# nyu-systems/Grendel-GS

Hardware: AMD Instinct MI355X
Metric: training iters/sec (fwd+bwd) (higher is better)
Workload: dtype f32

## Files before the change

### grendel-gs_amd/csrc/api.hip

```cpp
#include "common.h"

extern "C" {

const char *gsr_error_string(int code) {
    if (code == 0) return "success";
    if (code == GSR_EINVAL) return "gsraster: invalid argument";
    if (code == GSR_ENOSPACE) return "gsraster: workspace too small";
    if (code == GSR_ERETRY) return "gsraster: pair count valid, bounded sort must be repeated";
    if (code == GSR_EFAULT)
        return "gsraster: a persistent binning kernel of an earlier call timed out at a grid barrier (hung or preempted "
               "device); that view's lists are incomplete; the look-back pipeline is used from now on";
    if (code > 0) return hipGetErrorString((hipError_t)code);
    return "gsraster: unknown error";
}

int gsr_abi_version(void) { return 15; }

int gsr_get_block_xy(int *block_x, int *block_y, int *one_dim_block) {
    if (!block_x || !block_y || !one_dim_block) return GSR_EINVAL;
    *block_x = GSR_BLOCK_X;
    *block_y = GSR_BLOCK_Y;
    *one_dim_block = GSR_ONE_DIM_BLOCK;
    return 0;
}
// ... 98 lines not shown
    if (!xyz || !scaling || !rotation || !features_dc || !features_rest || !opacity || !viewmatrix || !projmatrix ||
        !campos || !radii || !cov3D || !clamped || !dL_dmeans2D || !dL_dconic_opacity || !dL_drgb || !dL_dxyz ||
        !dL_dscaling || !dL_drotation || !dL_dfeatures_dc || !dL_dfeatures_rest || !dL_dopacity)
        return GSR_EINVAL;
    return gsr_launch_preprocess_backward(P, sh_degree, sh_coeffs, xyz, scaling, scale_modifier, rotation, features_dc,
                                          features_rest, opacity, viewmatrix, projmatrix, campos, width, height,
                                          tanfovx, tanfovy, radii, cov3D, clamped, dL_dmeans2D, dL_dconic_opacity,
                                          dL_drgb, grad_row_stride, dL_dxyz, dL_dscaling, dL_drotation, dL_dfeatures_dc,
                                          dL_dfeatures_rest, dL_dopacity, gsr_antialiasing_mode(),
                                          reinterpret_cast<hipStream_t>(stream));
}

int gsr_get_local2j_ids_bool(int P, int width, int height, int world_size, const float *means2D,
                             const int32_t *radii, const int32_t *dist_global_strategy, uint8_t *out,
                             gsr_stream_t stream) {
    if (P < 0 || width <= 0 || height <= 0 || world_size <= 0) return GSR_EINVAL;
    if (P == 0) return 0;
    if (!means2D || !radii || !dist_global_strategy || !out) return GSR_EINVAL;
    return gsr_launch_local2j(P, width, height, world_size, means2D, radii, dist_global_strategy, out,
                              reinterpret_cast<hipStream_t>(stream));
}

size_t gsr_render_seg_bytes(int width, int height) {
    if (width <= 0 || height <= 0) return 0;
    return gsr_composite_seg_bytes(width, height);
}

int gsr_render_forward(int P, int width, int height, const int32_t *ranges, const uint32_t *point_list,
                       const float *means2D, const float *conic_opacity, const float *rgb,
                       const uint8_t *compute_locally, const float *bg, float *out_color, float *final_T,
                       int32_t *n_contrib, void *seg_ws, size_t seg_bytes, int row_lo, int row_hi, void *zero_ptr,
                       size_t zero_bytes, gsr_stream_t stream) {
    if (P < 0 || width <= 0 || height <= 0) return GSR_EINVAL;
    if (!ranges || !compute_locally || !bg || !out_color || !final_T || !n_contrib) return GSR_EINVAL;
    if (P > 0 && (!means2D || !conic_opacity || !rgb)) return GSR_EINVAL;
    return gsr_launch_composite_forward(P, width, height, ranges, point_list, means2D, conic_opacity, rgb,
                                        compute_locally, bg, out_color, final_T, n_contrib, seg_ws, seg_bytes, row_lo,
                                        row_hi, zero_ptr, zero_bytes, reinterpret_cast<hipStream_t>(stream));
}

int gsr_render_backward(int P, int width, int height, const int32_t *ranges, const uint32_t *point_list,
                        const float *means2D, const float *conic_opacity, const float *rgb,
                        const uint8_t *compute_locally, const float *bg, const float *final_T,
                        const int32_t *n_contrib, const float *dL_dpixels, float *dL_record, const float *out_color,
                        void *seg_ws, size_t seg_bytes, int row_lo, int row_hi, int record_is_zero, double *acc64,
                        uint8_t *touched, gsr_stream_t stream) {
    if (P < 0 || width <= 0 || height <= 0) return GSR_EINVAL;
    if (P == 0) return 0;
    if (!ranges || !compute_locally || !bg || !final_T || !n_contrib || !dL_dpixels || !means2D || !conic_opacity ||
        !rgb || !dL_record || !acc64)
        return GSR_EINVAL;
    return gsr_launch_composite_backward(P, width, height, ranges, point_list, means2D, conic_opacity, rgb,
                                         compute_locally, bg, final_T, n_contrib, dL_dpixels, dL_record, out_color,
                                         seg_ws, seg_bytes, row_lo, row_hi, record_is_zero ? 1 : 0, acc64, touched,
                                         reinterpret_cast<hipStream_t>(stream));
}

int gsr_render_contrib(int P, int width, int height, const int32_t *ranges, const uint32_t *point_list,
                       const float *means2D, const float *conic_opacity, const uint8_t *compute_locally,
                       const int32_t *n_contrib, int row_lo, int row_hi, int64_t *hits, float *wmax, double *wsum,
                       gsr_stream_t stream) {
    if (P < 0 || width <= 0 || height <= 0) return GSR_EINVAL;
    if (P == 0) return 0;
    if (!ranges || !means2D || !conic_opacity || !compute_locally || !n_contrib || !hits || !wmax || !wsum)
        return GSR_EINVAL;
    return gsr_launch_composite_contrib(P, width, height, ranges, point_list, means2D, conic_opacity, compute_locally,
                                        n_contrib, row_lo, row_hi, hits, wmax, wsum,
                                        reinterpret_cast<hipStream_t>(stream));
}

int gsr_contrib_merge_rows(int64_t n, const int32_t *idx, const int64_t *src_hits, const float *src_wmax,
                           const double *src_wsum, int64_t *dst_hits, float *dst_wmax, double *dst_wsum,
                           gsr_stream_t stream) {
    if (n < 0) return GSR_EINVAL;
    if (n == 0) return 0;
    if (!idx || !src_hits || !src_wmax || !src_wsum || !dst_hits || !dst_wmax || !dst_wsum) return GSR_EINVAL;
    return gsr_launch_contrib_merge_rows(n, idx, src_hits, src_wmax, src_wsum, dst_hits, dst_wmax, dst_wsum,
                                         reinterpret_cast<hipStream_t>(stream));
}

int gsr_render_invdepth(int P, int width, int height, const int32_t *ranges, const uint32_t *point_list,
                        const float *means2D, const float *conic_opacity, const float *depths,
                        const uint8_t *compute_locally, const int32_t *n_contrib, int row_lo, int row_hi,
                        float *invdepth, gsr_stream_t stream) {
    if (P < 0 || width <= 0 || height <= 0 || !invdepth) return GSR_EINVAL;
    if (P > 0 && (!ranges || !means2D || !conic_opacity || !depths || !compute_locally || !n_contrib)) return GSR_EINVAL;
    return gsr_launch_composite_invdepth(P, width, height, ranges, point_list, means2D, conic_opacity, depths,
                                         compute_locally, n_contrib, row_lo, row_hi, invdepth,
                                         reinterpret_cast<hipStream_t>(stream));
}

int gsr_render_invdepth_backward(int P, int width, int height, const int32_t *ranges, const uint32_t *point_list,
                                 const float *means2D, const float *conic_opacity, const float *depths,
                                 const uint8_t *compute_locally, const int32_t *n_contrib, const float *final_T,
                                 const float *invdepth, const float *dL_dinvdepth, int row_lo, int row_hi,
                                 float *dL_record, double *acc64, gsr_stream_t stream) {
    if (P < 0 || width <= 0 || height <= 0) return GSR_EINVAL;
    if (P == 0) return 0;
    if (!ranges || !means2D || !conic_opacity || !depths || !compute_locally || !n_contrib || !final_T || !invdepth ||
        !dL_dinvdepth || !dL_record || !acc64)
        return GSR_EINVAL;
    return gsr_launch_composite_invdepth_backward(P, width, height, ranges, point_list, means2D, conic_opacity, depths,
                                                  compute_locally, n_contrib, final_T, dL_dinvdepth, row_lo, row_hi,
                                                  dL_record, acc64, reinterpret_cast<hipStream_t>(stream));
}

int gsr_depth_backward_means3d(int P, const int32_t *radii, const float *viewmatrix, const float *dL_ddepth,
// ... 10 lines not shown
```

### grendel-gs_amd/csrc/common.h

```cpp
#pragma once
#include <hip/hip_runtime.h>
#include <stdint.h>

#include "../../include/gsraster.h"

#define GSR_WAVE 64

#define GSR_LAUNCH_CHECK()                         \
    do {                                           \
        hipError_t e__ = hipGetLastError();        \
        if (e__ != hipSuccess) return (int)e__;    \
    } while (0)

#define GSR_HIP(expr)                              \
    do {                                           \
        hipError_t e__ = (expr);                   \
        if (e__ != hipSuccess) return (int)e__;    \
    } while (0)

static inline int gsr_div_up(long long a, long long b) { return (int)((a + b - 1) / b); }

__device__ __forceinline__ int gsr_xcd_span_of_block(int b, int nwg) {
#ifdef GSR_NO_XCD_MAP
    return b;
// ... 59 lines not shown
__device__ __forceinline__ bool gsr_can_touch_box(const float2 xy, const float4 co, float x0, float y0, float x1,
                                                  float y1) {
    if (!(co.w >= 1.0f / 255.0f)) return false;
    const float lim = (2.0f * 0.6931471805599453f) * __builtin_amdgcn_logf(255.0f * co.w) * 1.002f + 0.01f;
    const float l = x0 - xy.x, r = x1 - xy.x, t = y0 - xy.y, bt = y1 - xy.y;
    if (l <= 0.f && r >= 0.f && t <= 0.f && bt >= 0.f) return true;
    if (!(co.x > 0.f && co.z > 0.f)) return true;
    const float rcz = __builtin_amdgcn_rcpf(co.z), rcx = __builtin_amdgcn_rcpf(co.x);
    float q = gsr_edge_min_q(co.x, co.y, co.z, rcz, l, t, bt);
    q = fminf(q, gsr_edge_min_q(co.x, co.y, co.z, rcz, r, t, bt));
    q = fminf(q, gsr_edge_min_q(co.z, co.y, co.x, rcx, t, l, r));
    q = fminf(q, gsr_edge_min_q(co.z, co.y, co.x, rcx, bt, l, r));
    return !(q > lim);
}

__device__ __forceinline__ void gsr_adam1(float &p, float g, float &m, float &v, float lr_c, float b1, float b2,
                                          float omb1, float omb2, float inv_sqrt_bc2, float eps) {
    m = __builtin_fmaf(b1, m, __fmul_rn(omb1, g));
    v = __builtin_fmaf(b2, v, __fmul_rn(__fmul_rn(omb2, g), g));
    const float denom = __builtin_fmaf(__fsqrt_rn(v), inv_sqrt_bc2, eps);
    p = __builtin_fmaf(-lr_c, __fdiv_rn(m, denom), p);
}

int gsr_launch_preprocess_forward(int P, int D, int M, const float *means3D, const float *scales, float scale_modifier,
                                  const float *rotations, const float *shs, const float *shs_rest,
                                  const float *opacities,
                                  const float *viewmatrix, const float *projmatrix, const float *campos, int W, int H,
                                  float tanfovx, float tanfovy, float *means2D, float *depths, int32_t *radii,
                                  float *cov3D, float *conic_opacity, float *rgb, uint8_t *clamped, int aa,
                                  hipStream_t stream);
int gsr_launch_preprocess_backward(int P, int D, int M, const float *means3D, const float *scales,
                                   float scale_modifier, const float *rotations, const float *shs,
                                   const float *shs_rest, const float *opacities_raw, const float *viewmatrix, const float *projmatrix, const float *campos, int W,
                                   int H, float tanfovx, float tanfovy, const int32_t *radii, const float *cov3D,
                                   const uint8_t *clamped, const float *dL_dmeans2D, const float *dL_dconic_opacity,
                                   const float *dL_drgb, int grad_row_stride, float *dL_dmeans3D, float *dL_dscales, float *dL_drotations,
                                   float *dL_dshs, float *dL_dshs_rest, float *dL_dopacities, int aa,
                                   hipStream_t stream);
int gsr_antialiasing_mode();
int gsr_launch_local2j(int P, int W, int H, int ws, const float *means2D, const int32_t *radii, const int32_t *div,
                       uint8_t *out, hipStream_t stream);

int gsr_launch_composite_forward(int P, int W, int H, const int32_t *ranges, const uint32_t *point_list,
                                 const float *means2D, const float *conic_opacity, const float *rgb,
                                 const uint8_t *compute_locally, const float *bg, float *out_color, float *final_T,
                                 int32_t *n_contrib, void *seg_ws, size_t seg_bytes, int row_lo, int row_hi,
                                 void *zero_ptr, size_t zero_bytes, hipStream_t stream);
size_t gsr_composite_seg_bytes(int W, int H);
int gsr_launch_composite_backward(int P, int W, int H, const int32_t *ranges, const uint32_t *point_list,
                                  const float *means2D, const float *conic_opacity, const float *rgb,
                                  const uint8_t *compute_locally, const float *bg, const float *final_T,
                                  const int32_t *n_contrib, const float *dL_dpixels, float *dL_record,
                                  const float *out_color, void *seg_ws, size_t seg_bytes, int row_lo, int row_hi,
                                  int record_is_zero, double *acc64, uint8_t *touched, hipStream_t stream);
int gsr_launch_composite_contrib(int P, int W, int H, const int32_t *ranges, const uint32_t *point_list,
                                 const float *means2D, const float *conic_opacity, const uint8_t *compute_locally,
                                 const int32_t *n_contrib, int row_lo, int row_hi, int64_t *hits, float *wmax,
                                 double *wsum, hipStream_t stream);
int gsr_launch_contrib_merge_rows(int64_t n, const int32_t *idx, const int64_t *src_hits, const float *src_wmax,
                                  const double *src_wsum, int64_t *dst_hits, float *dst_wmax, double *dst_wsum,
                                  hipStream_t stream);
int gsr_launch_composite_invdepth(int P, int W, int H, const int32_t *ranges, const uint32_t *point_list,
                                  const float *means2D, const float *conic_opacity, const float *depths,
                                  const uint8_t *compute_locally, const int32_t *n_contrib, int row_lo, int row_hi,
                                  float *invdepth, hipStream_t stream);
int gsr_launch_composite_invdepth_backward(int P, int W, int H, const int32_t *ranges, const uint32_t *point_list,
                                           const float *means2D, const float *conic_opacity, const float *depths,
                                           const uint8_t *compute_locally, const int32_t *n_contrib,
                                           const float *final_T, const float *dL_dinvdepth, int row_lo, int row_hi,
                                           float *dL_record, double *acc64, hipStream_t stream);
int gsr_launch_depth_to_means3D(int P, const int32_t *radii, const float *viewmatrix, const float *dL_ddepth,
                                int row_stride, float *dL_dmeans3D, int overwrite, hipStream_t stream);
```

### grendel-gs_amd/csrc/composite.hip

```cpp
#include "common.h"
#include "composite_math.h"

namespace {

__device__ unsigned long long g_walked[2];

#ifdef GSR_STATS
__device__ unsigned long long g_stats[8];
#define GSR_STAT(i, v) do { const unsigned long long sv__ = (unsigned long long)(v); if (lane == 0) atomicAdd(&g_stats[i], sv__); } while (0)
#else
#define GSR_STAT(i, v) do { } while (0)
#endif

typedef float v2f __attribute__((ext_vector_type(2)));
constexpr int PREC = 20;
struct PairRec {
    v2f x, y, a2, b2, c2, o, r, g, b;
};
__device__ __forceinline__ void pair_store(float *__restrict__ slab, int pos, const Entry &e, float r, float g, float b) {
    float *rec = slab + (pos >> 1) * PREC + (pos & 1);
    rec[0] = e.x;  rec[2] = e.y;  rec[4] = e.a2;  rec[6] = e.b2;  rec[8] = e.c2;
    rec[10] = e.o; rec[12] = r;   rec[14] = g;    rec[16] = b;
}
__device__ __forceinline__ void pair_store_last(float *__restrict__ slab, int pos, int last) {
    slab[(pos >> 1) * PREC + 18 + (pos & 1)] = __int_as_float(last);
}
__device__ __forceinline__ PairRec pair_load_last(const float *__restrict__ slab, int pair, int &la, int &lb) {
    const float4 *q = reinterpret_cast<const float4 *>(slab + pair * PREC);
    const float4 q0 = q[0], q1 = q[1], q2 = q[2], q3 = q[3], q4 = q[4];
    PairRec p;
    p.x = v2f{q0.x, q0.y};  p.y = v2f{q0.z, q0.w};  p.a2 = v2f{q1.x, q1.y};  p.b2 = v2f{q1.z, q1.w};
    p.c2 = v2f{q2.x, q2.y}; p.o = v2f{q2.z, q2.w};  p.r = v2f{q3.x, q3.y};   p.g = v2f{q3.z, q3.w};
    p.b = v2f{q4.x, q4.y};
    la = __float_as_int(q4.z);
    lb = __float_as_int(q4.w);
    asm("" : "+v"(la), "+v"(lb));
    return p;
}
#ifdef GSR_LOG2O
#define GSR_PAD_O (-__builtin_inff())
#else
#define GSR_PAD_O 0.f
#endif
__device__ __forceinline__ PairRec pair_load(const float *__restrict__ slab, int pair) {
    const float4 *q = reinterpret_cast<const float4 *>(slab + pair * PREC);
    const float4 q0 = q[0], q1 = q[1], q2 = q[2], q3 = q[3];
    const float2 q4 = *reinterpret_cast<const float2 *>(q + 4);
    PairRec p;
    p.x = v2f{q0.x, q0.y};  p.y = v2f{q0.z, q0.w};  p.a2 = v2f{q1.x, q1.y};  p.b2 = v2f{q1.z, q1.w};
    p.c2 = v2f{q2.x, q2.y}; p.o = v2f{q2.z, q2.w};  p.r = v2f{q3.x, q3.y};   p.g = v2f{q3.z, q3.w};
    p.b = v2f{q4.x, q4.y};
    return p;
// ... 727 lines not shown

int gsr_launch_composite_forward(int P, int W, int H, const int32_t *ranges, const uint32_t *point_list,
                                 const float *means2D, const float *conic_opacity, const float *rgb,
                                 const uint8_t *compute_locally, const float *bg, float *out_color, float *final_T,
                                 int32_t *n_contrib, void *seg_ws, size_t seg_bytes, int row_lo, int row_hi,
                                 void *zero_ptr, size_t zero_bytes, hipStream_t stream) {
    (void)P;
    if (zero_bytes && (!zero_ptr || ((uintptr_t)zero_ptr & 15) || (zero_bytes & 3))) return GSR_EINVAL;
    const size_t zero16_n = zero_bytes / 16;
    if (zero_bytes & 15)
        GSR_HIP(hipMemsetAsync(reinterpret_cast<char *>(zero_ptr) + zero16_n * 16, 0, zero_bytes & 15, stream));
    const int gx = (W + GSR_BLOCK_X - 1) / GSR_BLOCK_X, gy = (H + GSR_BLOCK_Y - 1) / GSR_BLOCK_Y;
    const BandGrid b = band_grid_of(row_lo, row_hi, gx, gy);
    if (seg_ws && seg_bytes < seg_ws_bytes(gx * gy, SEG_CAP)) return GSR_ENOSPACE;
    const SegWs seg = seg_ws_of(seg_ws, gx * gy, SEG_CAP);
    if (seg_ws) GSR_HIP(hipMemsetAsync(seg_ws, 0, 64, stream));
    auto launch = [&](auto kern) {
        hipLaunchKernelGGL(kern, dim3(b.band ? b.band_tiles : gx * gy), dim3(256), 0, stream, W, H, gx,
                           reinterpret_cast<const int2 *>(ranges), point_list, reinterpret_cast<const float2 *>(means2D),
                           reinterpret_cast<const float4 *>(conic_opacity), rgb, compute_locally, bg, out_color, final_T,
                           n_contrib, seg, b.band_first, b.band_tiles, reinterpret_cast<uint4 *>(zero_ptr), zero16_n);
    };
    if (seg_ws && b.band) launch(composite_forward_kernel<true, true>);
    else if (seg_ws) launch(composite_forward_kernel<true, false>);
    else if (b.band) launch(composite_forward_kernel<false, true>);
    else launch(composite_forward_kernel<false, false>);
    GSR_LAUNCH_CHECK();
    return 0;
}

__global__ void record_from_f64_kernel(const double *__restrict__ acc, float *__restrict__ rec, size_t n) {
    const size_t i = (size_t)blockIdx.x * blockDim.x + threadIdx.x;
    if (i < n) rec[i] = (float)acc[i];
}

__global__ void record_from_f64_touched_kernel(const double *__restrict__ acc, float *__restrict__ rec,
                                               const uint8_t *__restrict__ touched, int P) {
    const int i = (int)(blockIdx.x * blockDim.x + threadIdx.x);
    if (i >= P || !touched[i]) return;
    const double *a = acc + 9 * (size_t)i;
    float *r = rec + 9 * (size_t)i;
    double v[9];
#pragma unroll
    for (int k = 0; k < 9; k++) v[k] = a[k];
#pragma unroll
    for (int k = 0; k < 9; k++) r[k] = (float)v[k];
}

int gsr_launch_composite_backward(int P, int W, int H, const int32_t *ranges, const uint32_t *point_list,
                                  const float *means2D, const float *conic_opacity, const float *rgb,
                                  const uint8_t *compute_locally, const float *bg, const float *final_T,
                                  const int32_t *n_contrib, const float *dL_dpixels, float *dL_record,
                                  const float *out_color, void *seg_ws, size_t seg_bytes, int row_lo, int row_hi,
                                  int record_is_zero, double *acc64, uint8_t *touched, hipStream_t stream) {
    if (!record_is_zero) {
        touched = nullptr;
        GSR_HIP(hipMemsetAsync(acc64, 0, sizeof(double) * 9 * (size_t)P, stream));
    }
    if (P == 0) return 0;
    const int gx = (W + GSR_BLOCK_X - 1) / GSR_BLOCK_X, gy = (H + GSR_BLOCK_Y - 1) / GSR_BLOCK_Y;
    const BandGrid b = band_grid_of(row_lo, row_hi, gx, gy);
    if (seg_ws && (seg_bytes < seg_ws_bytes(gx * gy, SEG_CAP) || !out_color)) return GSR_EINVAL;
    const SegWs seg = seg_ws_of(seg_ws, gx * gy, SEG_CAP);
    if (seg_ws) GSR_HIP(hipMemsetAsync(reinterpret_cast<char *>(seg_ws) + sizeof(uint32_t), 0, sizeof(uint32_t), stream));
    const dim3 grid((b.band ? b.band_tiles : gx * gy) + (seg_ws ? SEG_WORKERS : 0));
    hipLaunchKernelGGL(composite_backward_kernel, grid, dim3(256), 0, stream, W, H, gx, gx * gy,
                       reinterpret_cast<const int2 *>(ranges), point_list, reinterpret_cast<const float2 *>(means2D),
                       reinterpret_cast<const float4 *>(conic_opacity), rgb, compute_locally, bg, final_T, n_contrib,
                       dL_dpixels, acc64, seg, b.band_first, b.band_tiles, touched);
    GSR_LAUNCH_CHECK();
    if (touched)
        hipLaunchKernelGGL(record_from_f64_touched_kernel, dim3((unsigned)((P + 255) / 256)), dim3(256), 0, stream,
                           acc64, dL_record, touched, P);
    else
        hipLaunchKernelGGL(record_from_f64_kernel, dim3((unsigned)((9 * (size_t)P + 255) / 256)), dim3(256), 0, stream,
                           acc64, dL_record, 9 * (size_t)P);
    GSR_LAUNCH_CHECK();
    return 0;
}
```

### grendel-gs_amd/csrc/preprocess.hip

```cpp
#include "common.h"

#include <atomic>
#include <initializer_list>
#include <type_traits>

#pragma clang fp contract(off)

namespace {

__constant__ const float SH_C0 = 0.28209479177387814f;
__constant__ const float SH_C1 = 0.4886025119029199f;
__constant__ const float SH_C2[5] = {1.0925484305920792f, -1.0925484305920792f, 0.31539156525252005f,
                                     -1.0925484305920792f, 0.5462742152960396f};
__constant__ const float SH_C3[7] = {-0.5900435899266435f, 2.890611442640554f, -0.4570457994644658f,
                                     0.3731763325901154f, -0.4570457994644658f, 1.445305721320277f,
                                     -0.5900435899266435f};

struct Cam {
    float v[16];
    float p[16];
    float c[3];
};

__device__ __forceinline__ Cam load_cam(const float *__restrict__ view, const float *__restrict__ proj,
// ... 682 lines not shown
                p4[k] = vf4{pa[0], pa[1], pa[2], pa[3]};
                __builtin_nontemporal_store(vf4{ma[0], ma[1], ma[2], ma[3]}, m4 + k);
                __builtin_nontemporal_store(vf4{va[0], va[1], va[2], va[3]}, v4 + k);
            }
        }
    }
    for (int k = (nw & ~3) + threadIdx.x; k < nw; k += K11_BLOCK) {
        const size_t o = row0 * REST_W + k;
        float p = param[o], m = ad.m[t][o], v = ad.v[t][o];
        gsr_adam1(p, __fmul_rn(s_rest[k], gs), m, v, lr_c, b1, b2, omb1, omb2, isb, eps);
        param[o] = p;
        ad.m[t][o] = m;
        ad.v[t][o] = v;
    }
}

struct K11In {
    int32_t rad;
    float p[3], sc[3], dc[3], op;
    float4 q;
    float cv[6];
    float4 gco;
    float2 g2;
    float grgb[3];
    uint8_t cl[3];
};
template <bool RAW, bool AA = false>
__device__ __forceinline__ K11In k11_load(size_t i, const float *__restrict__ means3D, const float *__restrict__ scales,
                                          const float *__restrict__ rotations, const float *__restrict__ shs,
                                          const float *__restrict__ opacities_raw, const int32_t *__restrict__ radii,
                                          const float *__restrict__ cov3D, const uint8_t *__restrict__ clamped,
                                          const float *__restrict__ dL_dmeans2D,
                                          const float *__restrict__ dL_dconic_opacity,
                                          const float *__restrict__ dL_drgb, int gstride) {
    K11In in;
    in.rad = radii[i];
#pragma unroll
    for (int e = 0; e < 3; e++) {
        in.p[e] = means3D[3 * i + e];
        in.sc[e] = scales[3 * i + e];
        in.dc[e] = RAW ? shs[3 * i + e] : 0.f;
        in.cl[e] = clamped[3 * i + e];
        in.grgb[e] = dL_drgb[(gstride ? gstride : 3) * i + e];
    }
    in.op = (RAW || AA) ? opacities_raw[i] : 0.f;
    in.q = *reinterpret_cast<const float4 *>(rotations + 4 * i);
#pragma unroll
    for (int e = 0; e < 6; e++) in.cv[e] = cov3D[6 * i + e];
    in.gco = grad_ld4(dL_dconic_opacity, i, gstride);
    in.g2 = grad_ld2(dL_dmeans2D, i, gstride);
    return in;
}

template <bool RAW, bool ADAM>
__device__ __forceinline__ void k11_opacity_out(float op, float g, const int i, float (&sp)[14], float (&sg)[14],
                                                float *__restrict__ dL_dopacities) {
    if (ADAM) {
        const float so = sigmoidf(op);
        sp[13] = op;
        sg[13] = g * so * (1.0f - so);
    } else if (RAW) {
        const float so = sigmoidf(op);
        dL_dopacities[i] = g * so * (1.0f - so);
    } else {
        dL_dopacities[i] = g;
    }
}

template <int DEG, bool RAW, bool ADAM = false, bool AA = false>
__device__ __forceinline__ void
preprocess_backward_body(const K11In &in, float (&sp)[14], float (&sg)[14], const int i,
                         const float *__restrict__ rest_in, float *__restrict__ rest_out, int M, float scale_modifier,
                         const float *__restrict__ shs, const float *__restrict__ view, const float *__restrict__ proj,
                         const float *__restrict__ campos, int W, int H, float tanfovx, float tanfovy,
                         float *__restrict__ dL_dmeans3D, float *__restrict__ dL_dscales,
                         float4 *__restrict__ dL_drotations, float *__restrict__ dL_dshs,
                         float *__restrict__ dL_dopacities) {
    constexpr int NC = (DEG + 1) * (DEG + 1);
    float *dsh_out = dL_dshs + (size_t)i * M * 3;

    if (ADAM && in.rad <= 0) {
#pragma unroll
        for (int e = 0; e < 3; e++) {
            sp[e] = in.p[e];
            sp[3 + e] = in.sc[e];
            sp[10 + e] = in.dc[e];
        }
        sp[6] = in.q.x; sp[7] = in.q.y; sp[8] = in.q.z; sp[9] = in.q.w;
        sp[13] = in.op;
#pragma unroll
        for (int e = 0; e < 14; e++) sg[e] = 0.f;
        float *rp = rest_out;
        for (int k = 0; k < (M - 1) * 3; k++) rp[k] = 0.f;
        return;
    }
    if (RAW && in.rad <= 0) {
        dL_dmeans3D[3 * (size_t)i] = dL_dmeans3D[3 * (size_t)i + 1] = dL_dmeans3D[3 * (size_t)i + 2] = 0.f;
        dL_dscales[3 * (size_t)i] = dL_dscales[3 * (size_t)i + 1] = dL_dscales[3 * (size_t)i + 2] = 0.f;
        dL_drotations[i] = make_float4(0.f, 0.f, 0.f, 0.f);
        dL_dopacities[i] = 0.f;
        dL_dshs[3 * (size_t)i] = dL_dshs[3 * (size_t)i + 1] = dL_dshs[3 * (size_t)i + 2] = 0.f;
        float *rp = rest_out;
        for (int k = 0; k < (M - 1) * 3; k++) rp[k] = 0.f;
        return;
    }
    if (in.rad <= 0) {
// ... 99 lines not shown
            sg[6] = dq.x; sg[7] = dq.y; sg[8] = dq.z; sg[9] = dq.w;
        } else {
#pragma unroll
            for (int r = 0; r < 3; r++) dL_dscales[3 * (size_t)i + r] = gsc[r];
            dL_drotations[i] = dq;
        }
    }
}

template <int DEG, bool RAW, bool AA>
__global__ void __launch_bounds__(K11_BLOCK, K11_WAVES_PER_EU)
preprocess_backward_kernel(int P, int M, const float *__restrict__ means3D, const float *__restrict__ scales,
                           float scale_modifier, const float *__restrict__ rotations, const float *__restrict__ shs,
                           const float *__restrict__ shs_rest, const float *__restrict__ opacities_raw,
                           const float *__restrict__ view, const float *__restrict__ proj,
                           const float *__restrict__ campos, int W, int H, float tanfovx, float tanfovy,
                           const int32_t *__restrict__ radii, const float *__restrict__ cov3D,
                           const uint8_t *__restrict__ clamped, const float *__restrict__ dL_dmeans2D,
                           const float *__restrict__ dL_dconic_opacity, const float *__restrict__ dL_drgb, int gstride,
                           float *__restrict__ dL_dmeans3D, float *__restrict__ dL_dscales,
                           float4 *__restrict__ dL_drotations, float *__restrict__ dL_dshs,
                           float *__restrict__ dL_dshs_rest, float *__restrict__ dL_dopacities) {
    const int i = blockIdx.x * blockDim.x + threadIdx.x;
    float ad[14], ad2[14];
    const size_t ic = (size_t)min(i, P - 1);
    if constexpr (RAW) {
        __shared__ float s_rest[K11_BLOCK * REST_W];
        if (M == 16) {
            RestStage st = rest_stage_issue(shs_rest, P);
            const K11In in = k11_load<RAW, AA>(ic, means3D, scales, rotations, shs, opacities_raw, radii, cov3D, clamped,
                                               dL_dmeans2D, dL_dconic_opacity, dL_drgb, gstride);
            __builtin_amdgcn_sched_barrier(0);
            rest_stage_commit(s_rest, st, shs_rest, P);
            __syncthreads();
            if (i < P)
                preprocess_backward_body<DEG, RAW, false, AA>(in, ad, ad2, i, s_rest + threadIdx.x * REST_W,
                                                              s_rest + threadIdx.x * REST_W, M, scale_modifier, shs,
                                                              view, proj, campos, W, H, tanfovx, tanfovy, dL_dmeans3D,
                                                              dL_dscales, dL_drotations, dL_dshs, dL_dopacities);
            __syncthreads();
            rest_stage_out(s_rest, dL_dshs_rest, P);
            return;
        }
    }
    if (i >= P) return;
    const K11In in = k11_load<RAW, AA>(ic, means3D, scales, rotations, shs, opacities_raw, radii, cov3D, clamped,
                                       dL_dmeans2D, dL_dconic_opacity, dL_drgb, gstride);
    preprocess_backward_body<DEG, RAW, false, AA>(in, ad, ad2, i, RAW ? shs_rest + (size_t)i * (M - 1) * 3 : nullptr,
                                                  RAW ? dL_dshs_rest + (size_t)i * (M - 1) * 3 : nullptr, M,
                                                  scale_modifier, shs, view, proj, campos, W, H, tanfovx, tanfovy,
                                                  dL_dmeans3D, dL_dscales, dL_drotations, dL_dshs, dL_dopacities);
}

template <int DEG, bool AA>
__global__ void __launch_bounds__(K11_BLOCK, K11_WAVES_PER_EU)
preprocess_backward_adam_kernel(int P, float *__restrict__ xyz, float *__restrict__ scaling, float scale_modifier,
                                float *__restrict__ rotation, float *__restrict__ f_dc, float *__restrict__ f_rest,
                                float *__restrict__ opacity, const float *__restrict__ view,
                                const float *__restrict__ proj, const float *__restrict__ campos, int W, int H,
                                float tanfovx, float tanfovy, const int32_t *__restrict__ radii,
                                const float *__restrict__ cov3D, const uint8_t *__restrict__ clamped,
                                const float *__restrict__ dL_dmeans2D, const float *__restrict__ dL_dconic_opacity,
                                const float *__restrict__ dL_drgb, int gstride, const K11Adam ad_in) {
    if (ad_in.skip && *ad_in.skip) return;
    const K11Adam ad = k11_adam_resolve(ad_in);
    const int i = blockIdx.x * blockDim.x + threadIdx.x;
    __shared__ float s_rest[K11_BLOCK * REST_W];
    const size_t ic = (size_t)min(i, P - 1);
    RestStage st = rest_stage_issue(f_rest, P);
    const K11In in = k11_load<true>(ic, xyz, scaling, rotation, f_dc, opacity, radii, cov3D, clamped, dL_dmeans2D,
                                    dL_dconic_opacity, dL_drgb, gstride);
    __builtin_amdgcn_sched_barrier(0);
    rest_stage_commit(s_rest, st, f_rest, P);
    __syncthreads();
    float sp[14], sg[14];
    if (i < P)
        preprocess_backward_body<DEG, true, true, AA>(in, sp, sg, i, s_rest + threadIdx.x * REST_W,
                                                      s_rest + threadIdx.x * REST_W, 16, scale_modifier, f_dc, view,
                                                      proj, campos, W, H, tanfovx, tanfovy, nullptr, nullptr, nullptr,
                                                      nullptr, nullptr);
    __syncthreads();
    rest_adam_out(s_rest, f_rest, ad, P);
    __syncthreads();
    k11_adam_small_lds(s_rest, ad, P, i, xyz, scaling, rotation, f_dc, opacity, sp, sg);
}

constexpr int CAM_STRIDE = 40;

__device__ __forceinline__ Cam load_cam_packed(const float *__restrict__ c) {
    Cam cam;
#pragma unroll
    for (int i = 0; i < 16; i++) {
        cam.v[i] = c[i];
        cam.p[i] = c[16 + i];
    }
    cam.c[0] = c[32];
    cam.c[1] = c[33];
    cam.c[2] = c[34];
    return cam;
}

template <int DEG, bool AA>
__global__ void __launch_bounds__(GSR_ONE_DIM_BLOCK)
preprocess_forward_batched_kernel(int P, int B, int M, const float *__restrict__ xyz, const float *__restrict__ scaling,
                                  float scale_modifier, const float *__restrict__ rotation,
                                  const float *__restrict__ f_dc, const float *__restrict__ f_rest,
                                  const float *__restrict__ opacity, const float *__restrict__ cams, int W, int H,
                                  float2 *__restrict__ means2D, float *__restrict__ depths,
                                  int32_t *__restrict__ radii, float *__restrict__ cov3D,
                                  float4 *__restrict__ conic_opacity, float *__restrict__ rgb,
                                  uint8_t *__restrict__ clamped) {
    const int i = blockIdx.x * blockDim.x + threadIdx.x;
    constexpr int NC = (DEG + 1) * (DEG + 1);
    if (i >= P) return;
    const int gx = (W + GSR_BLOCK_X - 1) / GSR_BLOCK_X, gy = (H + GSR_BLOCK_Y - 1) / GSR_BLOCK_Y;
    const float p[3] = {xyz[3 * (size_t)i], xyz[3 * (size_t)i + 1], xyz[3 * (size_t)i + 2]};
    float qnr, qn;
    const float4 q = quat_normalize(*reinterpret_cast<const float4 *>(rotation + 4 * (size_t)i), qnr, qn);
    const float s[3] = {scale_modifier * expf(scaling[3 * (size_t)i]), scale_modifier * expf(scaling[3 * (size_t)i + 1]),
                        scale_modifier * expf(scaling[3 * (size_t)i + 2])};
    const float op = sigmoidf(opacity[i]);
    float S[3][3];
    cov3d_from_scale_rot(q, s, S);
    cov3D[6 * (size_t)i + 0] = S[0][0]; cov3D[6 * (size_t)i + 1] = S[0][1]; cov3D[6 * (size_t)i + 2] = S[0][2];
    cov3D[6 * (size_t)i + 3] = S[1][1]; cov3D[6 * (size_t)i + 4] = S[1][2]; cov3D[6 * (size_t)i + 5] = S[2][2];
    float shl[NC * 3];
    shl[0] = f_dc[3 * (size_t)i];
    shl[1] = f_dc[3 * (size_t)i + 1];
    shl[2] = f_dc[3 * (size_t)i + 2];
    {
        const float *rp = f_rest + (size_t)i * (M - 1) * 3;
#pragma unroll
        for (int k = 3; k < NC * 3; k++) shl[k] = rp[k - 3];
    }
    for (int bc = 0; bc < B; bc++) {
        const float *cp = cams + (size_t)bc * CAM_STRIDE;
        const Cam cam = load_cam_packed(cp);
// ... 19 lines not shown
        } while (false);
        const size_t o = (size_t)bc * P + i;
        radii[o] = radius;
        means2D[o] = xy;
        depths[o] = depth;
        conic_opacity[o] = co;
#pragma unroll
        for (int k = 0; k < 3; k++) {
            rgb[3 * o + k] = col[k];
            clamped[3 * o + k] = cl[k] ? 1 : 0;
        }
    }
}

#ifndef GSR_K11_CAMQ
#define GSR_K11_CAMQ 2
#endif
constexpr int K11_CAMQ = GSR_K11_CAMQ;
#ifndef GSR_K11B_WAVES
#define GSR_K11B_WAVES 2
#endif
constexpr int K11B_WAVES_PER_EU = GSR_K11B_WAVES;
struct K11CamSH {
    int32_t rad;
    float grgb[3];
    uint8_t cl[3];
};
struct K11CamGeo {
    int32_t rad;
    float4 gco;
    float2 g2;
};
__device__ __forceinline__ K11CamSH k11_cam_load_sh(size_t o, const int32_t *__restrict__ radii,
                                                    const uint8_t *__restrict__ clamped,
                                                    const float *__restrict__ dL_drgb, int gstride) {
    K11CamSH c;
    c.rad = radii[o];
#pragma unroll
    for (int e = 0; e < 3; e++) {
        c.grgb[e] = dL_drgb[(gstride ? gstride : 3) * o + e];
        c.cl[e] = clamped[3 * o + e];
    }
    return c;
}
__device__ __forceinline__ K11CamGeo k11_cam_load_geo(size_t o, const int32_t *__restrict__ radii,
                                                      const float *__restrict__ dL_dmeans2D,
                                                      const float *__restrict__ dL_dconic_opacity, int gstride) {
    K11CamGeo c;
    c.rad = radii[o];
    c.gco = grad_ld4(dL_dconic_opacity, o, gstride);
    c.g2 = grad_ld2(dL_dmeans2D, o, gstride);
    return c;
}

struct DenseRows {};
struct ListRows {
    const uint32_t *list;
    uint32_t count;
};
constexpr int SA_UN = 5;
__device__ __forceinline__ size_t sa_rest_offset(const uint32_t *__restrict__ s_rows, int e) {
    const int r = e / REST_W;
    return (size_t)s_rows[r] * REST_W + (size_t)(e - r * REST_W);
}
__device__ __forceinline__ void sa_rest_stage_in(float *__restrict__ s_rest, const uint32_t *__restrict__ s_rows,
                                                 const float *__restrict__ f_rest, int nw) {
    for (int k0 = 0; k0 < REST_W; k0 += SA_UN) {
        float v[SA_UN];
#pragma unroll
        for (int u = 0; u < SA_UN; u++)
            v[u] = f_rest[sa_rest_offset(s_rows, min((k0 + u) * K11_BLOCK + (int)threadIdx.x, nw - 1))];
        __builtin_amdgcn_sched_barrier(0);
#pragma unroll
        for (int u = 0; u < SA_UN; u++) {
            const int e = (k0 + u) * K11_BLOCK + (int)threadIdx.x;
            if (e < nw) s_rest[e] = v[u];
        }
    }
}
__device__ __forceinline__ void sa_adam_small(const K11Adam &ad, size_t ic, float *__restrict__ xyz,
                                              float *__restrict__ scaling, float *__restrict__ rotation,
                                              float *__restrict__ f_dc, float *__restrict__ opacity,
                                              const float (&sp)[14], const float (&sg)[14]) {
    constexpr int T[14] = {0, 0, 0, 1, 1, 1, 2, 2, 2, 2, 3, 3, 3, 5};
    constexpr int KK[14] = {3, 3, 3, 3, 3, 3, 4, 4, 4, 4, 3, 3, 3, 1};
    constexpr int C[14] = {0, 1, 2, 0, 1, 2, 0, 1, 2, 3, 0, 1, 2, 0};
    float *const base[6] = {xyz, scaling, rotation, f_dc, nullptr, opacity};
    float m[14], v[14];
#pragma unroll
    for (int e = 0; e < 14; e++) {
        m[e] = ad.m[T[e]][ic * KK[e] + C[e]];
        v[e] = ad.v[T[e]][ic * KK[e] + C[e]];
    }
#pragma unroll
    for (int e = 0; e < 14; e++) {
        const int t = T[e];
        float pe = sp[e];
        gsr_adam1(pe, __fmul_rn(sg[e], ad.grad_scale), m[e], v[e], ad.lr_c[t], ad.b1[t], ad.b2[t], ad.omb1[t],
                  ad.omb2[t], ad.inv_sqrt_bc2[t], ad.eps[t]);
        base[t][ic * KK[e] + C[e]] = pe;
        ad.m[t][ic * KK[e] + C[e]] = m[e];
        ad.v[t][ic * KK[e] + C[e]] = v[e];
    }
}
__device__ __forceinline__ void sa_rest_adam_out(const float *__restrict__ s_rest, const uint32_t *__restrict__ s_rows,
                                                 float *__restrict__ f_rest, const K11Adam &ad, int nw) {
    constexpr int t = 4;
    float *const mr = ad.m[t], *const vr = ad.v[t];
    const float gs = ad.grad_scale, lr_c = ad.lr_c[t], b1 = ad.b1[t], b2 = ad.b2[t], omb1 = ad.omb1[t],
                omb2 = ad.omb2[t], isb = ad.inv_sqrt_bc2[t], eps = ad.eps[t];
    for (int k0 = 0; k0 < REST_W; k0 += SA_UN) {
        size_t off[SA_UN];
        float pn[SA_UN], mn[SA_UN], vn[SA_UN];
#pragma unroll
        for (int u = 0; u < SA_UN; u++) {
            off[u] = sa_rest_offset(s_rows, min((k0 + u) * K11_BLOCK + (int)threadIdx.x, nw - 1));
            pn[u] = f_rest[off[u]];
            mn[u] = mr[off[u]];
            vn[u] = vr[off[u]];
        }
        __builtin_amdgcn_sched_barrier(0);
#pragma unroll
        for (int u = 0; u < SA_UN; u++) {
            const int e = (k0 + u) * K11_BLOCK + (int)threadIdx.x;
            if (e < nw) {
                gsr_adam1(pn[u], __fmul_rn(s_rest[e], gs), mn[u], vn[u], lr_c, b1, b2, omb1, omb2, isb, eps);
                f_rest[off[u]] = pn[u];
                mr[off[u]] = mn[u];
                vr[off[u]] = vn[u];
            }
        }
    }
}

template <int DEG, bool ADAM, bool AA, typename ROWS = DenseRows>
__device__ __forceinline__ void
preprocess_backward_batched_body(int P, int B, int M, const float *__restrict__ xyz,
                                   const float *__restrict__ scaling, float scale_modifier,
                                   const float *__restrict__ rotation, const float *__restrict__ f_dc,
                                   const float *__restrict__ f_rest, const float *__restrict__ opacity,
                                   const float *__restrict__ cams, int W, int H, const int32_t *__restrict__ radii,
                                   const float *__restrict__ cov3D, const uint8_t *__restrict__ clamped,
                                   const float *__restrict__ dL_dmeans2D,
                                   const float *__restrict__ dL_dconic_opacity, const float *__restrict__ dL_drgb,
                                   int gstride,
                                   float *__restrict__ dL_dxyz, float *__restrict__ dL_dscaling,
                                   float4 *__restrict__ dL_drotation, float *__restrict__ dL_ddc,
                                   float *__restrict__ dL_drest, float *__restrict__ dL_dopacity, const K11Adam &ad,
                                   const ROWS rows = ROWS{}) {
    constexpr bool LIST = std::is_same<ROWS, ListRows>::value;
    static_assert(!LIST || ADAM, "ListRows is the sparse K11 + Adam update (and takes M == 16)");
    __shared__ float s_rest[K11_BLOCK * REST_W];
    __shared__ uint32_t s_rows[LIST ? K11_BLOCK : 1];
    const bool staged = M == 16;
    constexpr int NC = (DEG + 1) * (DEG + 1);
    int i, nrows = 0;
    size_t ic;
    RestStage st;
    if constexpr (LIST) {
        const size_t first = (size_t)blockIdx.x * K11_BLOCK;
        nrows = (int)min((size_t)K11_BLOCK, (size_t)rows.count - first);
        const uint32_t irow = rows.list[first + min((int)threadIdx.x, nrows - 1)];
        s_rows[threadIdx.x] = irow;
        i = (int)irow;
        ic = irow;
    } else {
        i = blockIdx.x * blockDim.x + threadIdx.x;
        ic = (size_t)min(i, P - 1);
        if (staged) st = rest_stage_issue(f_rest, P);
    }
    const float p[3] = {xyz[3 * ic], xyz[3 * ic + 1], xyz[3 * ic + 2]};
    float cvr[6];
#pragma unroll
    for (int e = 0; e < 6; e++) cvr[e] = cov3D[6 * ic + e];
    const float dc[3] = {f_dc[3 * ic], f_dc[3 * ic + 1], f_dc[3 * ic + 2]};
    const float oraw = opacity[ic];
    const float4 qraw = *reinterpret_cast<const float4 *>(rotation + 4 * ic);
    const float scraw[3] = {scaling[3 * ic], scaling[3 * ic + 1], scaling[3 * ic + 2]};
    K11CamSH shq[K11_CAMQ];
    K11CamGeo geoq[K11_CAMQ];
    if constexpr (!LIST) {
#pragma unroll
        for (int u = 0; u < K11_CAMQ; u++) {
            const size_t o = (size_t)min(u, B - 1) * P + ic;
            shq[u] = k11_cam_load_sh(o, radii, clamped, dL_drgb, gstride);
            geoq[u] = k11_cam_load_geo(o, radii, dL_dmeans2D, dL_dconic_opacity, gstride);
        }
    }
    __builtin_amdgcn_sched_barrier(0);
    if constexpr (LIST) {
        __syncthreads();
        sa_rest_stage_in(s_rest, s_rows, f_rest, nrows * REST_W);
        __syncthreads();
    } else if (staged) {
        rest_stage_commit(s_rest, st, f_rest, P);
        __syncthreads();
    }
    float sp[14], sg[14];
    if (LIST ? (int)threadIdx.x < nrows : i < P) {
    float S[3][3];
    cov3d_unpack(cvr, S);
    const float *const shl = s_rest + threadIdx.x * REST_W;
    float sh[NC * 3];
    sh[0] = dc[0];
    sh[1] = dc[1];
    sh[2] = dc[2];
    if (!staged) {
        const float *rp = f_rest + (size_t)i * (M - 1) * 3;
#pragma unroll
        for (int k = 3; k < NC * 3; k++) sh[k] = rp[k - 3];
    }
    float dmean[3] = {0.f, 0.f, 0.f};
    float dcov[6] = {0.f, 0.f, 0.f, 0.f, 0.f, 0.f};
    float dsh[NC * 3];
#pragma unroll
    for (int k = 0; k < NC * 3; k++) dsh[k] = 0.f;
    float dop = 0.f;
    const float op_act = AA ? sigmoidf(oraw) : 0.f;

    for (int bc = 0; bc < B; bc++) {
        const K11CamSH cin = LIST ? k11_cam_load_sh((size_t)bc * P + ic, radii, clamped, dL_drgb, gstride) : shq[0];
        if constexpr (!LIST) {
#pragma unroll
            for (int u = 0; u + 1 < K11_CAMQ; u++) shq[u] = shq[u + 1];
            if (bc + K11_CAMQ < B)
                shq[K11_CAMQ - 1] = k11_cam_load_sh((size_t)(bc + K11_CAMQ) * P + i, radii, clamped, dL_drgb, gstride);
        }
        if (cin.rad <= 0) continue;
        if (staged) asm volatile("" ::: "memory");
        const float *cp = cams + (size_t)bc * CAM_STRIDE;
        const float camc[3] = {cp[32], cp[33], cp[34]};
        const float g3[3] = {cin.cl[0] ? 0.f : cin.grgb[0], cin.cl[1] ? 0.f : cin.grgb[1],
                             cin.cl[2] ? 0.f : cin.grgb[2]};
        float dm[3];
        viewdir_backward<DEG>(camc, p, ShStagedOrRegs{staged, shl, sh}, g3, DshAdd{dsh}, dm);
        dmean[0] += dm[0];
        dmean[1] += dm[1];
        dmean[2] += dm[2];
    }
    if constexpr (ADAM) {
#pragma unroll
        for (int e = 0; e < 3; e++) {
            sp[10 + e] = sh[e];
            sg[10 + e] = dsh[e];
        }
    } else {
        dL_ddc[3 * (size_t)i] = dsh[0];
        dL_ddc[3 * (size_t)i + 1] = dsh[1];
        dL_ddc[3 * (size_t)i + 2] = dsh[2];
    }
    {
        float *rp = staged ? s_rest + threadIdx.x * REST_W : dL_drest + (size_t)i * (M - 1) * 3;
#pragma unroll
        for (int k = 3; k < NC * 3; k++) rp[k - 3] = dsh[k];
        for (int k = NC * 3; k < M * 3; k++) rp[k - 3] = 0.f;
    }
    for (int bc = 0; bc < B; bc++) {
        const K11CamGeo cin =
            LIST ? k11_cam_load_geo((size_t)bc * P + ic, radii, dL_dmeans2D, dL_dconic_opacity, gstride) : geoq[0];
        if constexpr (!LIST) {
#pragma unroll
            for (int u = 0; u + 1 < K11_CAMQ; u++) geoq[u] = geoq[u + 1];
            if (bc + K11_CAMQ < B)
                geoq[K11_CAMQ - 1] = k11_cam_load_geo((size_t)(bc + K11_CAMQ) * P + i, radii, dL_dmeans2D,
                                                      dL_dconic_opacity, gstride);
        }
        if (cin.rad <= 0) continue;
        const float *cp = cams + (size_t)bc * CAM_STRIDE;
        const Cam cam = load_cam_packed(cp);
        const float tanfovx = cp[35], tanfovy = cp[36];
        const float fx = W / (2.0f * tanfovx), fy = H / (2.0f * tanfovy);
        const float4 gco = cin.gco;
        const float gA = gco.x, gB = gco.y, gC = gco.z;
        if (!AA) dop += gco.w;
        const Cov2DGrad cg = cov2d_backward<AA>(cam.v, fx, fy, tanfovx, tanfovy, p, S, gA, gB, gC,
                                                AA ? gco.w * op_act : 0.f);
        if (AA) dop += gco.w * cg.rho;
        if (cg.live) {
#pragma unroll
            for (int e = 0; e < 6; e++) dcov[e] += cg.dcov[e];
        }
#pragma unroll
        for (int k = 0; k < 3; k++) dmean[k] += cg.dmean[k];
        float dm[3];
        means2d_to_mean(cam.p, p, cin.g2, dm);
#pragma unroll
        for (int k = 0; k < 3; k++) dmean[k] += dm[k];
    }
    if constexpr (ADAM) {
#pragma unroll
        for (int e = 0; e < 3; e++) {
            sp[e] = p[e];
            sg[e] = dmean[e];
        }
    } else {
        dL_dxyz[3 * (size_t)i] = dmean[0];
        dL_dxyz[3 * (size_t)i + 1] = dmean[1];
        dL_dxyz[3 * (size_t)i + 2] = dmean[2];
    }
    {
        const float so = sigmoidf(oraw);
        if constexpr (ADAM) {
            sp[13] = oraw;
            sg[13] = dop * so * (1.0f - so);
        } else {
            dL_dopacity[i] = dop * so * (1.0f - so);
        }
    }
    {
        float gsc[3];
        float4 gq;
        cov3d_backward<true>(qraw, scraw, scale_modifier, dcov, gsc, gq);
        if constexpr (ADAM) {
#pragma unroll
            for (int e = 0; e < 3; e++) {
                sp[3 + e] = scraw[e];
                sg[3 + e] = gsc[e];
            }
// ... 11 lines not shown
    }
    if constexpr (LIST) {
        __syncthreads();
        sa_rest_adam_out(s_rest, s_rows, const_cast<float *>(f_rest), ad, nrows * REST_W);
    } else if (staged) {
        __syncthreads();
        if constexpr (ADAM) {
            rest_adam_out(s_rest, const_cast<float *>(f_rest), ad, P);
            __syncthreads();
            k11_adam_small_lds(s_rest, ad, P, i, const_cast<float *>(xyz), const_cast<float *>(scaling),
                               const_cast<float *>(rotation), const_cast<float *>(f_dc), const_cast<float *>(opacity),
                               sp, sg);
        } else {
            rest_stage_out(s_rest, dL_drest, P);
        }
    }
}

template <int DEG, bool AA>
__global__ void __launch_bounds__(K11_BLOCK, K11B_WAVES_PER_EU)
preprocess_backward_batched_kernel(int P, int B, int M, const float *__restrict__ xyz,
                                   const float *__restrict__ scaling, float scale_modifier,
                                   const float *__restrict__ rotation, const float *__restrict__ f_dc,
                                   const float *__restrict__ f_rest, const float *__restrict__ opacity,
                                   const float *__restrict__ cams, int W, int H, const int32_t *__restrict__ radii,
                                   const float *__restrict__ cov3D, const uint8_t *__restrict__ clamped,
                                   const float *__restrict__ dL_dmeans2D,
                                   const float *__restrict__ dL_dconic_opacity, const float *__restrict__ dL_drgb,
                                   int gstride, float *__restrict__ dL_dxyz, float *__restrict__ dL_dscaling,
                                   float4 *__restrict__ dL_drotation, float *__restrict__ dL_ddc,
                                   float *__restrict__ dL_drest, float *__restrict__ dL_dopacity) {
    preprocess_backward_batched_body<DEG, false, AA>(P, B, M, xyz, scaling, scale_modifier, rotation, f_dc, f_rest,
                                                     opacity, cams, W, H, radii, cov3D, clamped, dL_dmeans2D,
                                                     dL_dconic_opacity, dL_drgb, gstride, dL_dxyz, dL_dscaling,
                                                     dL_drotation, dL_ddc, dL_drest, dL_dopacity, K11Adam{});
}

template <int DEG, bool AA>
__global__ void __launch_bounds__(K11_BLOCK, K11B_WAVES_PER_EU)
preprocess_backward_adam_batched_kernel(int P, int B, float *__restrict__ xyz, float *__restrict__ scaling,
                                        float scale_modifier, float *__restrict__ rotation,
                                        float *__restrict__ f_dc, float *__restrict__ f_rest,
                                        float *__restrict__ opacity, const float *__restrict__ cams, int W, int H,
                                        const int32_t *__restrict__ radii, const float *__restrict__ cov3D,
                                        const uint8_t *__restrict__ clamped, const float *__restrict__ dL_dmeans2D,
                                        const float *__restrict__ dL_dconic_opacity,
                                        const float *__restrict__ dL_drgb, int gstride, const K11Adam ad_in) {
    if (ad_in.skip && *ad_in.skip) return;
    const K11Adam ad = k11_adam_resolve(ad_in);
    preprocess_backward_batched_body<DEG, true, AA>(P, B, 16, xyz, scaling, scale_modifier, rotation, f_dc, f_rest,
                                                    opacity, cams, W, H, radii, cov3D, clamped, dL_dmeans2D,
                                                    dL_dconic_opacity, dL_drgb, gstride, nullptr, nullptr, nullptr,
                                                    nullptr, nullptr, nullptr, ad);
}

constexpr int SA_CBLOCK = 256;
constexpr int SA_CPER = 4;
constexpr int SA_CROWS = SA_CBLOCK * SA_CPER;
struct SparseWs {
    uint32_t count, pad[3];
};

__device__ __forceinline__ bool sa_nonzero(float x) {
    return (__float_as_uint(x) & 0x7fffffffu) != 0u;
}

__global__ void sparse_adam_reset_kernel(const uint32_t *__restrict__ skip, SparseWs *__restrict__ ws) {
    if (skip && *skip) return;
    ws->count = 0u;
}

__global__ void __launch_bounds__(SA_CBLOCK)
sparse_adam_classify_kernel(int P, int B, const int32_t *__restrict__ radii, const float *__restrict__ dL_dmeans2D,
                            const float *__restrict__ dL_dconic_opacity, const float *__restrict__ dL_drgb, int gstride,
                            const uint32_t *__restrict__ skip, SparseWs *__restrict__ ws, uint32_t *__restrict__ list,
                            uint8_t *__restrict__ active_out) {
    if (skip && *skip) return;
    constexpr int NW = SA_CBLOCK / GSR_WAVE;
    __shared__ uint32_t s_cnt[SA_CPER * NW];
    __shared__ uint32_t s_base;
    const size_t row0 = (size_t)blockIdx.x * SA_CROWS;
    const int wave = threadIdx.x / GSR_WAVE;
    bool act[SA_CPER];
    uint32_t rank[SA_CPER];
#pragma unroll
    for (int j = 0; j < SA_CPER; j++) {
        const size_t i = row0 + (size_t)j * SA_CBLOCK + threadIdx.x;
        bool a = false;
        if (i < (size_t)P) {
            for (int bc = 0; bc < B; bc++) {
                const size_t o = (size_t)bc * P + i;
                if (radii[o] <= 0) continue;
                const float2 g2 = grad_ld2(dL_dmeans2D, o, gstride);
                const float4 gco = grad_ld4(dL_dconic_opacity, o, gstride);
                const float *gr = dL_drgb + (size_t)(gstride ? gstride : 3) * o;
                a = a || sa_nonzero(g2.x) || sa_nonzero(g2.y) || sa_nonzero(gr[0]) || sa_nonzero(gr[1]) ||
                    sa_nonzero(gr[2]) || sa_nonzero(gco.x) || sa_nonzero(gco.y) || sa_nonzero(gco.z) ||
                    sa_nonzero(gco.w);
            }
            if (active_out) active_out[i] = a ? 1 : 0;
        }
        const unsigned long long bal = __ballot(a);
        act[j] = a;
        rank[j] = __builtin_amdgcn_mbcnt_hi((uint32_t)(bal >> 32), __builtin_amdgcn_mbcnt_lo((uint32_t)bal, 0u));
        if ((threadIdx.x & (GSR_WAVE - 1)) == 0) s_cnt[j * NW + wave] = (uint32_t)__popcll(bal);
    }
// ... 316 lines not shown
                                                   const int32_t *radii, const float *cov3D, const uint8_t *clamped,
                                                   const float *dL_dmeans2D, const float *dL_dconic_opacity,
                                                   const float *dL_drgb, int grad_row_stride, float *dL_dxyz, float *dL_dscaling,
                                                   float *dL_drotation, float *dL_dfeatures_dc,
                                                   float *dL_dfeatures_rest, float *dL_dopacity, gsr_stream_t stream) {
    if (P < 0 || B < 1 || sh_degree < 0 || sh_degree > 3 || sh_coeffs < 2 ||
        sh_coeffs < (sh_degree + 1) * (sh_degree + 1) || width <= 0 || height <= 0)
        return GSR_EINVAL;
    if (P == 0) return 0;
    if (!xyz || !scaling || !rotation || !features_dc || !features_rest || !opacity || !cams || !radii || !cov3D ||
        !clamped || !dL_dmeans2D || !dL_dconic_opacity || !dL_drgb || !dL_dxyz || !dL_dscaling || !dL_drotation ||
        !dL_dfeatures_dc || !dL_dfeatures_rest || !dL_dopacity)
        return GSR_EINVAL;
    const dim3 grid(gsr_div_up(P, K11_BLOCK)), block(K11_BLOCK);
    GSR_DISPATCH_DEG_AA(sh_degree, gsr_antialiasing_mode(),
                     hipLaunchKernelGGL((preprocess_backward_batched_kernel<DEG, AA>), grid, block, 0,
                                        reinterpret_cast<hipStream_t>(stream), P, B, sh_coeffs, xyz, scaling,
                                        scale_modifier, rotation, features_dc, features_rest, opacity, cams, width,
                                        height, radii, cov3D, clamped, dL_dmeans2D, dL_dconic_opacity, dL_drgb,
                                        grad_row_stride, dL_dxyz,
                                        dL_dscaling, reinterpret_cast<float4 *>(dL_drotation), dL_dfeatures_dc,
                                        dL_dfeatures_rest, dL_dopacity));
    GSR_LAUNCH_CHECK();
    return 0;
}

static bool k11_adam_fill(K11Adam &ad, std::initializer_list<const void *> device_arrays, float *const *exp_avgs,
                          float *const *exp_avg_sqs, const double *lrs, const double *beta1s, const double *beta2s,
                          const double *epss, const int64_t *steps, float grad_scale, const float *dyn_dev,
                          const uint32_t *skip_flag_dev) {
    for (const void *a : device_arrays)
        if (!a) return true;
    if (!exp_avgs || !exp_avg_sqs || !beta1s || !beta2s || !epss || (!dyn_dev && (!lrs || !steps))) return true;
    ad.dyn = dyn_dev;
    ad.skip = skip_flag_dev;
    ad.grad_scale = grad_scale;
    for (int t = 0; t < 6; t++) {
        if (!exp_avgs[t] || !exp_avg_sqs[t] || (!dyn_dev && steps[t] < 1)) return true;
        const double bc1 = dyn_dev ? 1.0 : 1.0 - pow(beta1s[t], (double)steps[t]);
        const double bc2 = dyn_dev ? 1.0 : 1.0 - pow(beta2s[t], (double)steps[t]);
        ad.m[t] = exp_avgs[t];
        ad.v[t] = exp_avg_sqs[t];
        ad.lr_c[t] = dyn_dev ? 0.f : (float)(lrs[t] / bc1);
        ad.b1[t] = (float)beta1s[t];
        ad.b2[t] = (float)beta2s[t];
        ad.omb1[t] = (float)(1.0 - beta1s[t]);
        ad.omb2[t] = (float)(1.0 - beta2s[t]);
        ad.inv_sqrt_bc2[t] = (float)(1.0 / sqrt(bc2));
        ad.eps[t] = (float)epss[t];
    }
    return false;
}

extern "C" int gsr_preprocess_backward_adam_raw_batched(
    int P, int B, int sh_degree, int sh_coeffs, float *xyz, float *scaling, float scale_modifier, float *rotation,
    float *features_dc, float *features_rest, float *opacity, const float *cams, int width, int height,
    const int32_t *radii, const float *cov3D, const uint8_t *clamped, const float *dL_dmeans2D,
    const float *dL_dconic_opacity, const float *dL_drgb, int grad_row_stride, float *const *exp_avgs,
    float *const *exp_avg_sqs, const double *lrs, const double *beta1s, const double *beta2s, const double *epss,
    const int64_t *steps, float grad_scale, const float *tanfov0, gsr_stream_t stream) {
    return gsr_preprocess_backward_adam_raw_batched_dyn(
        P, B, sh_degree, sh_coeffs, xyz, scaling, scale_modifier, rotation, features_dc, features_rest, opacity, cams,
        width, height, radii, cov3D, clamped, dL_dmeans2D, dL_dconic_opacity, dL_drgb, grad_row_stride, exp_avgs,
        exp_avg_sqs, lrs, beta1s, beta2s, epss, steps, grad_scale, tanfov0, nullptr, nullptr, stream);
}

extern "C" int gsr_preprocess_backward_adam_raw_batched_dyn(
    int P, int B, int sh_degree, int sh_coeffs, float *xyz, float *scaling, float scale_modifier, float *rotation,
    float *features_dc, float *features_rest, float *opacity, const float *cams, int width, int height,
    const int32_t *radii, const float *cov3D, const uint8_t *clamped, const float *dL_dmeans2D,
    const float *dL_dconic_opacity, const float *dL_drgb, int grad_row_stride, float *const *exp_avgs,
    float *const *exp_avg_sqs, const double *lrs, const double *beta1s, const double *beta2s, const double *epss,
    const int64_t *steps, float grad_scale, const float *tanfov0, const float *dyn_dev, const uint32_t *skip_flag_dev,
    gsr_stream_t stream) {
    if (P < 0 || B < 1 || sh_degree < 0 || sh_degree > 3 || sh_coeffs != 16 || width <= 0 || height <= 0)
        return GSR_EINVAL;
    if (P == 0) return 0;
    K11Adam ad{};
    if (k11_adam_fill(ad, {xyz, scaling, rotation, features_dc, features_rest, opacity, cams, radii, cov3D, clamped,
                           dL_dmeans2D, dL_dconic_opacity, dL_drgb},
                      exp_avgs, exp_avg_sqs, lrs, beta1s, beta2s, epss, steps, grad_scale, dyn_dev, skip_flag_dev))
        return GSR_EINVAL;
    uintptr_t al = (uintptr_t)features_rest | (uintptr_t)rotation;
    for (int t = 0; t < 6; t++) al |= (uintptr_t)ad.m[t] | (uintptr_t)ad.v[t];
    if (al & 15) return GSR_EINVAL;
    const dim3 grid(gsr_div_up(P, K11_BLOCK)), block(K11_BLOCK);
    const int aa = gsr_antialiasing_mode();
    if (B == 1 && tanfov0) {
        GSR_DISPATCH_DEG_AA(sh_degree, aa,
                         hipLaunchKernelGGL((preprocess_backward_adam_kernel<DEG, AA>), grid, block, 0,
                                            reinterpret_cast<hipStream_t>(stream), P, xyz, scaling, scale_modifier,
                                            rotation, features_dc, features_rest, opacity, cams, cams + 16, cams + 32,
                                            width, height, tanfov0[0], tanfov0[1], radii, cov3D, clamped, dL_dmeans2D,
                                            dL_dconic_opacity, dL_drgb, grad_row_stride, ad));
        GSR_LAUNCH_CHECK();
        return 0;
    }
    GSR_DISPATCH_DEG_AA(sh_degree, aa,
                     hipLaunchKernelGGL((preprocess_backward_adam_batched_kernel<DEG, AA>), grid, block, 0,
                                        reinterpret_cast<hipStream_t>(stream), P, B, xyz, scaling, scale_modifier,
                                        rotation, features_dc, features_rest, opacity, cams, width, height, radii,
                                        cov3D, clamped, dL_dmeans2D, dL_dconic_opacity, dL_drgb, grad_row_stride, ad));
    GSR_LAUNCH_CHECK();
    return 0;
}

extern "C" size_t gsr_sparse_step_workspace_bytes(int P) {
    return sizeof(SparseWs) + sizeof(uint32_t) * 2 * (((size_t)(P > 0 ? P : 1) + 1) / 2);
}

extern "C" int gsr_preprocess_backward_adam_raw_batched_sparse(
    int P, int B, int sh_degree, int sh_coeffs, float *xyz, float *scaling, float scale_modifier, float *rotation,
    float *features_dc, float *features_rest, float *opacity, const float *cams, int width, int height,
    const int32_t *radii, const float *cov3D, const uint8_t *clamped, const float *dL_dmeans2D,
    const float *dL_dconic_opacity, const float *dL_drgb, int grad_row_stride, float *const *exp_avgs,
    float *const *exp_avg_sqs, const double *lrs, const double *beta1s, const double *beta2s, const double *epss,
    const int64_t *steps, float grad_scale, const float *dyn_dev, const uint32_t *skip_flag_dev, void *workspace,
    size_t workspace_bytes, uint8_t *active_out, uint32_t *num_active_dev, gsr_stream_t stream) {
    if (P < 0 || B < 1 || sh_degree < 0 || sh_degree > 3 || sh_coeffs != 16 || width <= 0 || height <= 0 ||
        grad_row_stride < 0 || (grad_row_stride != 0 && grad_row_stride < 9))
        return GSR_EINVAL;
    if (P == 0) return 0;
    if (!workspace) return GSR_EINVAL;
    K11Adam ad{};
    if (k11_adam_fill(ad, {xyz, scaling, rotation, features_dc, features_rest, opacity, cams, radii, cov3D, clamped,
                           dL_dmeans2D, dL_dconic_opacity, dL_drgb},
                      exp_avgs, exp_avg_sqs, lrs, beta1s, beta2s, epss, steps, grad_scale, dyn_dev, skip_flag_dev))
        return GSR_EINVAL;
    if ((uintptr_t)rotation & 15) return GSR_EINVAL;
    if (grad_row_stride == 0 && (((uintptr_t)dL_dmeans2D & 7) || ((uintptr_t)dL_dconic_opacity & 15)))
        return GSR_EINVAL;
    if (((uintptr_t)workspace & 7) || workspace_bytes < gsr_sparse_step_workspace_bytes(P)) return GSR_ENOSPACE;
    hipStream_t st = reinterpret_cast<hipStream_t>(stream);
    SparseWs *ws = static_cast<SparseWs *>(workspace);
    uint32_t *list = reinterpret_cast<uint32_t *>(ws + 1);
    hipLaunchKernelGGL(sparse_adam_reset_kernel, dim3(1), dim3(1), 0, st, skip_flag_dev, ws);
    GSR_LAUNCH_CHECK();
    hipLaunchKernelGGL(sparse_adam_classify_kernel, dim3(gsr_div_up(P, SA_CROWS)), dim3(SA_CBLOCK), 0, st, P, B, radii,
                       dL_dmeans2D, dL_dconic_opacity, dL_drgb, grad_row_stride, skip_flag_dev, ws, list, active_out);
    GSR_LAUNCH_CHECK();
    const dim3 grid(gsr_div_up(P, K11_BLOCK)), block(K11_BLOCK);
    GSR_DISPATCH_DEG_AA(sh_degree, gsr_antialiasing_mode(),
                     hipLaunchKernelGGL((sparse_adam_update_kernel<DEG, AA>), grid, block, 0, st, P, B, xyz, scaling,
                                        scale_modifier, rotation, features_dc, features_rest, opacity, cams, width,
                                        height, radii, cov3D, clamped, dL_dmeans2D, dL_dconic_opacity, dL_drgb,
                                        grad_row_stride, ad, ws, list, num_active_dev));
    GSR_LAUNCH_CHECK();
    return 0;
}

extern "C" size_t gsr_preprocess_backward_cams_bytes(int P, int B) {
    const int nb = kc_blocks(P, 1);
    return (size_t)(nb > 0 ? nb : 1) * (size_t)(B > 0 ? B : 1) * KC_NS * sizeof(double);
}

extern "C" int gsr_preprocess_backward_cams(int P, int B, int sh_degree, int sh_coeffs, const float *means3D,
                                            const float *sh_dc, int sh_dc_stride, const float *sh_rest,
// ... 40 lines not shown
```

### grendel-gs_amd/diff_gaussian_rasterization/__init__.py

```python
import contextlib
import ctypes
import os
from typing import NamedTuple

import torch
import torch.nn as nn

from . import _lib
from ._lib import check, lib

__all__ = ["GaussianRasterizationSettings", "GaussianRasterizer", "_C", "load_image_tiles_by_pos",
           "merge_image_tiles_by_pos", "set_timing_mode", "fused_l1_ssim_band", "fused_band_loss", "fused_band_loss_exposure", "fused_activations", "pack_camera",
           "preprocess_gaussians_raw_batched", "knn_mean_dist2", "group_rows", "gather_rows", "densify_plan", "densify_move", "exchange_need",
           "exchange_count", "exchange_pack", "exchange_pack_slab", "exchange_unpack", "zeros_async", "scatter_add_rows", "densify_stats",
           "set_tie_order", "scatter_rows", "local_pixels", "GraphCapture", "capturing", "image_metrics", "metrics_from_sums"]

BLOCK_X, BLOCK_Y, ONE_DIM_BLOCK_SIZE = 16, 16, 256

_TIMING_MODE = "auto"
_last_backward_ms = 0.0


def set_timing_mode(mode):
    global _TIMING_MODE
    assert mode in ("auto", "sync", "stale", "deferred", "off")
    _TIMING_MODE = mode


def _timing_mode():
    if _TIMING_MODE != "auto":
        return _TIMING_MODE
    if torch.distributed.is_available() and torch.distributed.is_initialized() and \
            torch.distributed.get_world_size() > 1:
        return "sync"
    return "stale"


class _KernelTimer:

    def __init__(self):
        self.enabled = False
        self.records = {}

    class _Range:
        def __init__(self, owner, name, meta):
            self.owner, self.name, self.meta = owner, name, meta

        def __enter__(self):
            if self.owner.enabled:
                self.e0 = torch.cuda.Event(enable_timing=True)
                self.e1 = torch.cuda.Event(enable_timing=True)
                self.e0.record()
            return self

        def __exit__(self, *exc):
            if self.owner.enabled:
                self.e1.record()
                self.owner.records.setdefault(self.name, []).append((self.e0, self.e1, self.meta))

# ... 400 lines not shown
        return _PreprocessGaussians.forward(ctx, means3D, scales, rotations, shs, opacities, rs, cuda_args)

    @staticmethod
    def backward(ctx, g_means2D, g_rgb, g_conic_opacity, g_radii, g_depths):
        means3D, scales, rotations, shs, view, proj, campos, radii, cov3D, clamped = ctx.saved_tensors
        g_means2D, g_rgb, g_conic_opacity, gstride = _grad_triple(g_means2D, g_rgb, g_conic_opacity,
                                                                  means3D.shape[0], means3D.device)
        d_cam = _single_camera_grads(ctx, means3D, shs, view, proj, campos, radii, cov3D, clamped, g_means2D,
                                     g_conic_opacity, g_rgb, gstride)
        return _PreprocessGaussians.backward(ctx, g_means2D, g_rgb, g_conic_opacity, g_radii, g_depths)[:5] + \
            d_cam + (None, None)


class _PreprocessGaussiansRawCam(torch.autograd.Function):

    @staticmethod
    def forward(ctx, xyz, scaling, rotation, features_dc, features_rest, opacity, viewmatrix, projmatrix, campos,
                raster_settings, cuda_args):
        _refuse_camera_grad_under_antialiasing("preprocess_gaussians_raw")
        ctx.cam_slot = 6
        ctx.cam_like = [(t.dtype, t.shape) for t in (viewmatrix, projmatrix, campos)]
        rs = raster_settings._replace(viewmatrix=viewmatrix, projmatrix=projmatrix, campos=campos)
        return _PreprocessGaussiansRaw.forward(ctx, xyz, scaling, rotation, features_dc, features_rest, opacity, rs,
                                               cuda_args)

    @staticmethod
    def backward(ctx, g_means2D, g_rgb, g_conic_opacity, g_radii, g_depths):
        xyz, scaling, rotation, f_dc, f_rest, opacity, view, proj, campos, radii, cov3D, clamped = ctx.saved_tensors
        g_means2D, g_rgb, g_conic_opacity, gstride = _grad_triple(g_means2D, g_rgb, g_conic_opacity, xyz.shape[0],
                                                                  xyz.device)
        d_cam = _single_camera_grads(ctx, xyz, (f_dc, f_rest), view, proj, campos, radii, cov3D, clamped, g_means2D,
                                     g_conic_opacity, g_rgb, gstride)
        return _PreprocessGaussiansRaw.backward(ctx, g_means2D, g_rgb, g_conic_opacity, g_radii, g_depths)[:6] + \
            d_cam + (None, None)


def _batched_record(grads, B, P):
    g0 = grads[0]
    if g0 is None or g0._base is None:
        return None
    base = g0._base
    if base.dtype != torch.float32 or not base.is_contiguous() or base.numel() != B * P * 9:
        return None
    p0 = base.data_ptr()
    for k in range(B):
        for col, (off, cols) in enumerate(((0, 2), (2, 3), (5, 4))):
            g = grads[5 * k + col]
            if g is None or g._base is not base or tuple(g.shape) != (P, cols) or g.stride() != (9, 1) or \
                    g.data_ptr() != p0 + 4 * (k * P * 9 + off):
                return None
    return base.view(B * P, 9)


_DEFERRED_SINK = [None]


def set_deferred_backward_sink(sink):
    import weakref

    _DEFERRED_SINK[0] = weakref.ref(sink) if sink is not None else None


def deferred_backward_sink():
    ref = _DEFERRED_SINK[0]
    return ref() if ref is not None else None


class PendingProjectionBackward:

    def __init__(self, params, cams, radii, cov3D, clamped, g_means2D, g_conic_opacity, g_rgb, gstride, meta, tanfov0):
        self.params = params
        self.versions = tuple(t._version for t in params)
        self.cams, self.radii, self.cov3D, self.clamped = cams, radii, cov3D, clamped
        self.g_means2D, self.g_conic_opacity, self.g_rgb, self.gstride = g_means2D, g_conic_opacity, g_rgb, gstride
        self.meta, self.tanfov0 = meta, tanfov0
        self.stream = current_stream(params[0].device) if params[0].is_cuda else None

    def join_stream(self):
        if self.stream is not None:
            cur = current_stream(self.params[0].device)
            if cur != self.stream:
                cur.wait_stream(self.stream)

    def materialize(self):
        self.join_stream()
        return _launch_k11(self.params, self.cams, self.radii, self.cov3D, self.clamped, self.g_means2D,
                           self.g_conic_opacity, self.g_rgb, self.gstride, self.meta, self.tanfov0, None)

    def fused_step(self, exp_avgs, exp_avg_sqs, lrs, beta1s, beta2s, epss, steps, grad_scale, cache=None,
                   sparse=False):
        self.join_stream()
        xyz, scaling, rotation, f_dc, f_rest, opacity = self.params
        deg, smod, W, H, M = self.meta[:5]
        P, B = xyz.shape[0], self.cams.shape[0]
        VP, D, I64 = ctypes.c_void_p * 6, ctypes.c_double * 6, ctypes.c_int64 * 6
        key = (tuple(t.data_ptr() for t in exp_avgs), tuple(t.data_ptr() for t in exp_avg_sqs), tuple(beta1s),
               tuple(beta2s), tuple(epss))
        tabs = cache.get("tabs") if cache is not None else None
        if tabs is None or tabs[0] != key:
            tabs = (key, VP(*key[0]), VP(*key[1]), D(*beta1s), D(*beta2s), D(*epss))
            if cache is not None:
                cache["tabs"] = tabs
        tf = (ctypes.c_float * 2)(float(self.tanfov0[0]), float(self.tanfov0[1])) \
            if (B == 1 and self.tanfov0 is not None) else None
        cap_ctx = _CAPTURE[0]
        dyn, flag = (_ptr(cap_ctx.dyn), _ptr(cap_ctx.flag)) if cap_ctx is not None else (None, None)
        args = [P, B, deg, M, _ptr(xyz), _ptr(scaling), smod, _ptr(rotation), _ptr(f_dc), _ptr(f_rest), _ptr(opacity),
                _ptr(self.cams), W, H, _ptr(self.radii), _ptr(self.cov3D), _ptr(self.clamped), _ptr(self.g_means2D),
                _ptr(self.g_conic_opacity), _ptr(self.g_rgb), self.gstride, tabs[1], tabs[2],
                None if cap_ctx is not None else D(*lrs), tabs[3], tabs[4], tabs[5],
                None if cap_ctx is not None else I64(*steps), float(grad_scale)]
        if sparse:
            if cache is None:
                cache = {}
            need = int(lib.gsr_sparse_step_workspace_bytes(P))
            ws = cache.get("sparse_ws")
            if ws is None or ws[0] != P or ws[1].device != xyz.device or ws[1].numel() * 8 < need:
                ws = (P, torch.empty((need + 7) // 8, dtype=torch.int64, device=xyz.device),
                      torch.zeros(1, dtype=torch.int32, device=xyz.device))
                cache["sparse_ws"] = ws
                cache["num_active"] = ws[2]
            name, timed = "gsr_preprocess_backward_adam_raw_batched_sparse", "preprocess_backward_adam_sparse"
            args += [dyn, flag, _ptr(ws[1]), ws[1].numel() * 8, None, _ptr(ws[2])]
        elif cap_ctx is not None:
            name, timed = "gsr_preprocess_backward_adam_raw_batched_dyn", None
            args += [tf, dyn, flag]
        else:
            name, timed = "gsr_preprocess_backward_adam_raw_batched", "preprocess_backward_adam"
            args += [tf]
        _lib_antialiasing(_meta_aa(self.meta))
        with _on(xyz.device), (kernel_timer.range(timed, N=P, B=B, M=M) if cap_ctx is None else _NULL_RANGE):
            check(getattr(lib, name)(*args, _stream()), name)


def _launch_k11(params, cams, radii, cov3D, clamped, g_means2D, g_conic_opacity, g_rgb, gstride, meta, tanfov0,
                cuda_args_list):
    xyz, scaling, rotation, f_dc, f_rest, opacity = params
    deg, smod, W, H, M = meta[:5]
    _lib_antialiasing(_meta_aa(meta))
    P, B = xyz.shape[0], cams.shape[0]
    dev = xyz.device
    d_xyz = torch.empty((P, 3), dtype=torch.float32, device=dev)
    d_scaling = torch.empty((P, 3), dtype=torch.float32, device=dev)
    d_rot = torch.empty((P, 4), dtype=torch.float32, device=dev)
    d_dc = torch.empty((P, 1, 3), dtype=torch.float32, device=dev)
    d_rest = torch.empty((P, M - 1, 3), dtype=torch.float32, device=dev)
    d_opac = torch.empty((P, 1), dtype=torch.float32, device=dev)
    with _on(dev), kernel_timer.range("preprocess_backward", N=P, B=B, M=M), \
            zhx_range(cuda_args_list, "b20 preprocess time"):
        if B == 1 and tanfov0 is not None:
            base = cams.data_ptr()
            check(lib.gsr_preprocess_backward_raw(
                P, deg, M, _ptr(xyz), _ptr(scaling), smod, _ptr(rotation), _ptr(f_dc), _ptr(f_rest),
                _ptr(opacity), ctypes.c_void_p(base), ctypes.c_void_p(base + 64), ctypes.c_void_p(base + 128), W,
                H, float(tanfov0[0]), float(tanfov0[1]), _ptr(radii), _ptr(cov3D), _ptr(clamped),
                _ptr(g_means2D), _ptr(g_conic_opacity), _ptr(g_rgb), gstride, _ptr(d_xyz), _ptr(d_scaling),
                _ptr(d_rot), _ptr(d_dc), _ptr(d_rest), _ptr(d_opac), _stream()), "gsr_preprocess_backward_raw")
        else:
            check(lib.gsr_preprocess_backward_raw_batched(
                P, B, deg, M, _ptr(xyz), _ptr(scaling), smod, _ptr(rotation), _ptr(f_dc), _ptr(f_rest),
                _ptr(opacity), _ptr(cams), W, H, _ptr(radii), _ptr(cov3D), _ptr(clamped), _ptr(g_means2D),
                _ptr(g_conic_opacity), _ptr(g_rgb), gstride, _ptr(d_xyz), _ptr(d_scaling), _ptr(d_rot),
                _ptr(d_dc), _ptr(d_rest), _ptr(d_opac), _stream()), "gsr_preprocess_backward_raw_batched")
    return d_xyz, d_scaling, d_rot, d_dc, d_rest, d_opac


class _PreprocessGaussiansRawBatched(torch.autograd.Function):

    @staticmethod
    def forward(ctx, xyz, scaling, rotation, features_dc, features_rest, opacity, cams, sh_degree, scale_modifier,
                width, height, tanfov0, cuda_args_list=None):
        xyz, scaling, rotation = _f32c(xyz, "xyz"), _f32c(scaling, "scaling"), _f32c(rotation, "rotation")
        features_dc, features_rest = _f32c(features_dc, "features_dc"), _f32c(features_rest, "features_rest")
        opacity, cams = _f32c(opacity, "opacity"), _f32c(cams, "cams")
        ctx.tanfov0 = tanfov0
        ctx.cuda_args_list = cuda_args_list
        ctx.set_materialize_grads(False)
        P, B = xyz.shape[0], cams.shape[0]
        if cams.dim() != 2 or cams.shape[1] != 40:
            raise ValueError("cams must be [B, 40]")
        M = 1 + features_rest.shape[1]
        dev = xyz.device
        aa = _ANTIALIASING[0]
        if aa and ctx.needs_input_grad[6]:
            _refuse_camera_grad_under_antialiasing("preprocess_gaussians_raw_batched")
        _lib_antialiasing(aa)
        means2D = torch.empty((B, P, 2), dtype=torch.float32, device=dev)
        depths = torch.empty((B, P), dtype=torch.float32, device=dev)
        radii = torch.empty((B, P), dtype=torch.int32, device=dev)
        cov3D = torch.empty((P, 6), dtype=torch.float32, device=dev)
        conic_opacity = torch.empty((B, P, 4), dtype=torch.float32, device=dev)
        rgb = torch.empty((B, P, 3), dtype=torch.float32, device=dev)
        clamped = torch.empty((B, P, 3), dtype=torch.uint8, device=dev)
        with _on(dev), kernel_timer.range("preprocess_forward", N=P, B=B, M=M), \
                zhx_range(cuda_args_list, "10 preprocess time"):
            check(lib.gsr_preprocess_forward_raw_batched(
                P, B, int(sh_degree), M, _ptr(xyz), _ptr(scaling), float(scale_modifier), _ptr(rotation),
                _ptr(features_dc), _ptr(features_rest), _ptr(opacity), _ptr(cams), int(width), int(height),
                _ptr(means2D), _ptr(depths), _ptr(radii), _ptr(cov3D), _ptr(conic_opacity), _ptr(rgb), _ptr(clamped),
                _stream()), "gsr_preprocess_forward_raw_batched")
        ctx.meta = (int(sh_degree), float(scale_modifier), int(width), int(height), M, aa)
        ctx.save_for_backward(xyz, scaling, rotation, features_dc, features_rest, opacity, cams, radii, cov3D, clamped)
        outs = []
        for k in range(B):
            outs += [means2D[k], rgb[k], conic_opacity[k], radii[k], depths[k]]
        ctx.mark_non_differentiable(*[o for i, o in enumerate(outs) if i % 5 >= 3])
        return tuple(outs)

    @staticmethod
    def backward(ctx, *grads):
        xyz, scaling, rotation, f_dc, f_rest, opacity, cams, radii, cov3D, clamped = ctx.saved_tensors
        deg, smod, W, H, M = ctx.meta[:5]
        P, B = xyz.shape[0], cams.shape[0]
        dev = xyz.device

        def assemble(col, cols):
            gs = [grads[5 * k + col] for k in range(B)]
            if B == 1:
                return torch.zeros((1, P, cols), dtype=torch.float32, device=dev) if gs[0] is None \
                    else gs[0].float().contiguous()
            if all(g is not None and g.dtype == torch.float32 and g.is_contiguous() for g in gs):
                base, step = gs[0]._base, P * cols * 4
                if base is not None and all(g._base is base and g.data_ptr() == gs[0].data_ptr() + k * step
                                            for k, g in enumerate(gs)):
                    return gs[0]
            out = torch.zeros((B, P, cols), dtype=torch.float32, device=dev)
            for k, g in enumerate(gs):
                if g is not None:
                    out[k].copy_(g)
            return out

        if B == 1:
            g_means2D, g_rgb, g_conic_opacity, gstride = _grad_triple(grads[0], grads[1], grads[2], P, dev)
        else:
            rec = _batched_record(grads, B, P)
            if rec is not None:
                g_means2D, g_rgb, g_conic_opacity, gstride = rec[:, 0:2], rec[:, 2:5], rec[:, 5:9], 9
            else:
                g_means2D, g_rgb, g_conic_opacity, gstride = assemble(0, 2), assemble(1, 3), assemble(2, 4), 0
        params = (xyz, scaling, rotation, f_dc, f_rest, opacity)
        d_cams = None
        if ctx.needs_input_grad[6]:
            d_cams = preprocess_backward_cameras(xyz, (f_dc, f_rest), cams, W, H, deg, radii, cov3D, clamped,
                                                 g_means2D, g_conic_opacity, g_rgb, gstride)
        sink = deferred_backward_sink()
        if sink is not None and M == 16 and sink.accepts(params):
            sink.offer(PendingProjectionBackward(params, cams, radii, cov3D, clamped, g_means2D, g_conic_opacity,
                                                 g_rgb, gstride, ctx.meta, ctx.tanfov0))
            return (None,) * 6 + (d_cams,) + (None,) * 6
        return _launch_k11(params, cams, radii, cov3D, clamped, g_means2D, g_conic_opacity, g_rgb, gstride, ctx.meta,
                           ctx.tanfov0, ctx.cuda_args_list) + (d_cams,) + (None,) * 6


def preprocess_gaussians_raw_batched(xyz, scaling, rotation, features_dc, features_rest, opacity, cams, sh_degree,
                                     scale_modifier, width, height, tanfov0=None, cuda_args_list=None):
    flat = _PreprocessGaussiansRawBatched.apply(xyz, scaling, rotation, features_dc, features_rest, opacity, cams,
                                                sh_degree, scale_modifier, width, height, tanfov0, cuda_args_list)
    return tuple([flat[5 * k + c] for k in range(cams.shape[0])] for c in range(5))


def _bucket(nbytes):
    if nbytes < (1 << 20):
        return nbytes
    step = 1 << (int(nbytes).bit_length() - 4)
    return (nbytes + step - 1) // step * step


_SORT_SCRATCH = {}
_MAX_PAIRS = {}


def _sort_scratch(nbytes, dev):
    idx = dev.index if dev.index is not None else torch._C._cuda_getDevice()
    key = (idx, int(torch._C._cuda_getCurrentRawStream(idx)))
    buf = _SORT_SCRATCH.get(key)
    if buf is None or buf.numel() < nbytes:
        _SORT_SCRATCH.pop(key, None)
        buf = None
        buf = torch.empty((_bucket(nbytes),), dtype=torch.uint8, device=dev)
        _SORT_SCRATCH[key] = buf
    return buf


def release_workspaces():
    _SORT_SCRATCH.clear()
    _MAX_PAIRS.clear()


_SPECULATIVE_SORT = [os.environ.get("GSR_SPECULATIVE_SORT", "1") != "0"]
_SEGMENTS = [{"0": False, "always": "always"}.get(os.environ.get("GSR_SEGMENTS", "1"), True)]
_BAND_GRID = [os.environ.get("GSR_BAND_GRID", "1") != "0"]
_ZERO_IN_FORWARD = [os.environ.get("GSR_ZERO_IN_FORWARD", "1") != "0"]
_KEEP_BACKWARD_BUFFERS = [None]
_TOUCHED_ROWS = [os.environ.get("GSR_TOUCHED_ROWS", "1") != "0"]


def set_list_segments(on):
    _SEGMENTS[0] = "always" if on == "always" else bool(on)


def set_speculative_sort(on):
# ... 227 lines not shown
            mask = torch.ones((gy * gx,), dtype=torch.uint8, device=dev)
        else:
            if compute_locally.numel() != gx * gy:
                raise ValueError(f"compute_locally must have TILE_Y*TILE_X = {gy}x{gx} entries")
            mask = compute_locally.to(device=dev).contiguous().view(-1)
            mask = mask.view(torch.uint8) if mask.dtype == torch.bool else mask.to(torch.uint8)
        bg = _f32c(rs.bg, "bg")
        timing = (cuda_args.get("_gsr_timing") if isinstance(cuda_args, dict) else None) or _timing_mode()
        if _CAPTURE[0] is not None:
            timing = "off"
        stats = cuda_args.get("stats_collector") if isinstance(cuda_args, dict) else None
        contrib = cuda_args.get("contributions") if isinstance(cuda_args, dict) else None
        if contrib is not None:
            if _CAPTURE[0] is not None:
                raise RuntimeError("diff_gaussian_rasterization: cuda_args['contributions'] is not available under graph "
                                   "capture (the statistics need the view's final lists)")
            if not isinstance(contrib, ContributionStats) or contrib.P != P or \
                    contrib.hits.get_device() != means2D.get_device():
                raise ValueError(f"cuda_args['contributions'] must be a ContributionStats of {P} rows on {dev}")
        invd = bool(cuda_args.get("invdepth")) if isinstance(cuda_args, dict) else False
        if invd and _CAPTURE[0] is not None:
            raise RuntimeError("diff_gaussian_rasterization: cuda_args['invdepth'] is not available under graph capture "
                               "(the map needs the view's final lists)")
        with _on(dev):
            if timing != "off":
                ev0 = torch.cuda.Event(enable_timing=True)
                ev1 = torch.cuda.Event(enable_timing=True)
                ev0.record(current_stream(dev))
            if _CAPTURE[0] is not None:
                _CAPTURE[0].stamp("fwd0", id(stats))
            with kernel_timer.range("binning", P=P, tiles=gx * gy) as kt:
                point_list, ranges, D = bin_gaussians(means2D, depths, radii, conic_opacity, mask, W, H, cuda_args,
                                                      defer=contrib is None and not invd)
            pend = D if isinstance(D, PendingPairs) else None
            kt.meta["D"] = D = (0 if pend is not None else D)
            if kernel_timer.enabled:
                kt.meta["R"] = _LAST_SEGMENTS[0]
            out = torch.empty((3, H, W), dtype=torch.float32, device=dev)
            final_T = torch.empty((H, W), dtype=torch.float32, device=dev)
            n_contrib = torch.empty((H, W), dtype=torch.int32, device=dev)
            ctx.px_meta = dict(mask=mask, W=W, H=H) if kernel_timer.enabled else {}
            ctx.cuda_args = cuda_args
            band = cuda_args.get("_gsr_band") if (isinstance(cuda_args, dict) and _BAND_GRID[0]) else None
            row_lo, row_hi = (int(band[0]), int(band[1])) if band else (0, 0)
            band_rows = row_hi if row_lo == -1 else row_hi - row_lo
            thin = 0 < band_rows * gx <= 2048
            seg_ws, seg_bytes = None, 0
            if any(ctx.needs_input_grad[:3]) and (_SEGMENTS[0] == "always" or (_SEGMENTS[0] and thin)):
                seg_bytes = int(lib.gsr_render_seg_bytes(W, H))
                seg_ws = torch.empty((seg_bytes,), dtype=torch.uint8, device=dev)
            lists = [point_list]
            record = acc64 = touched = None
            zero_buf, zero_bytes = None, 0
            if any(ctx.needs_input_grad[:3]) and P > 0 and _ZERO_IN_FORWARD[0]:
                if _TOUCHED_ROWS[0]:
                    zero_bytes = 108 * P + ((P + 15) & ~15)
                    zero_buf = torch.empty((zero_bytes,), dtype=torch.uint8, device=dev)
                    acc64 = zero_buf[:72 * P].view(torch.float64).view(P, 9)
                    record = zero_buf[72 * P:108 * P].view(torch.float32).view(P, 9)
                    touched = zero_buf[108 * P:109 * P]
                else:
                    record = torch.empty((P, 9), dtype=torch.float32, device=dev)
                    zero_buf = acc64 = torch.empty((P, 9), dtype=torch.float64, device=dev)
                    zero_bytes = 72 * P
            ctx.record = (record, acc64, touched) if record is not None else None

            def launch_k8(meta_D):
                with kernel_timer.range("composite_forward", P=P, D=meta_D, **ctx.px_meta) as k8t, \
                        zhx_range(cuda_args, "70 render time"):
                    check(lib.gsr_render_forward(P, W, H, _ptr(ranges), _ptr(lists[0]), _ptr(means2D),
                                                 _ptr(conic_opacity), _ptr(rgb), _ptr(mask), _ptr(bg), _ptr(out),
                                                 _ptr(final_T), _ptr(n_contrib), _ptr(seg_ws), seg_bytes, row_lo,
                                                 row_hi, _ptr(zero_buf), zero_bytes, _stream()), "gsr_render_forward")
                return k8t

            k8t = launch_k8(D)
            if contrib is not None:
                contribution_stats(ranges, lists[0], means2D, conic_opacity, n_contrib, mask, W, H, contrib,
                                   band=(row_lo, row_hi))
            if invd:
                cuda_args[_INVDEPTH_KEY] = (ranges, lists[0], mask, (row_lo, row_hi), final_T, n_contrib, W, H)
            if _CAPTURE[0] is not None:
                _CAPTURE[0].stamp("fwd1", id(stats))
            ctx.seg = (seg_ws, seg_bytes, row_lo, row_hi)
            ctx.lists = lists
            ctx.num_rendered = D
            _RenderGaussians.last_num_rendered = D
            if pend is not None:
                def settle(ctx=ctx, pend=pend, kt=kt, k8t=k8t, lists=lists):
                    D, again = pend.finish()
                    kt.meta["D"] = k8t.meta["D"] = D
                    ctx.num_rendered = D
                    _RenderGaussians.last_num_rendered = D
                    if again is not None:
                        lists[0] = again
                        with _on(pend.dev), torch.cuda.stream(pend.stream):
                            launch_k8(D)
                    return D

                collector = cuda_args.get("_gsr_pending") if isinstance(cuda_args, dict) else None
                if isinstance(collector, list):
                    collector.append(settle)
                else:
                    settle()
            if timing != "off":
                ev1.record(current_stream(dev))
                ctx.fwd_events = (ev0, ev1)
        if stats is not None:
            stats.setdefault("forward_render_time", 0.0)
            stats.setdefault("backward_render_time", 0.0)
        ctx.raster_settings = rs
        ctx.cuda_args = cuda_args
        ctx.timing = timing
        ctx.save_for_backward(means2D, conic_opacity, rgb, mask, bg, ranges, final_T, n_contrib,
                              out if seg_ws is not None else None)
        ctx.mark_non_differentiable(n_contrib)
        return out, n_contrib

    @staticmethod
    def backward(ctx, g_out, _g_ncontrib):
        global _last_backward_ms
        rs = ctx.raster_settings
        means2D, conic_opacity, rgb, mask, bg, ranges, final_T, n_contrib, out_img = ctx.saved_tensors
        point_list = ctx.lists[0]
        H, W = int(rs.image_height), int(rs.image_width)
        P = means2D.shape[0]
        dev = means2D.device
        if g_out is None:
            return None, None, None, None, None, None, None, None, None
        g_out = g_out.float().contiguous()
        pair, ctx.record = ctx.record, None
        record_is_zero = pair is not None
        if pair is None:
            pair = (torch.empty((P, 9), dtype=torch.float32, device=dev),
                    torch.empty((P, 9), dtype=torch.float64, device=dev), None)
        record, acc64, touched = pair
        if _KEEP_BACKWARD_BUFFERS[0] is not None:
            _KEEP_BACKWARD_BUFFERS[0].append(pair)
        d_means2D, d_rgb, d_conic_opacity = record[:, 0:2], record[:, 2:5], record[:, 5:9]
        timing = ctx.timing
        with _on(dev):
            if timing != "off":
                ev0 = torch.cuda.Event(enable_timing=True)
                ev1 = torch.cuda.Event(enable_timing=True)
                ev0.record(current_stream(dev))
            cap_stats = ctx.cuda_args.get("stats_collector") if isinstance(ctx.cuda_args, dict) else None
            if _CAPTURE[0] is not None:
                _CAPTURE[0].stamp("bwd0", id(cap_stats))
            with kernel_timer.range("composite_backward", P=P, D=ctx.num_rendered, **ctx.px_meta), \
                    zhx_range(ctx.cuda_args, "b10 render time"):
                seg_ws, seg_bytes, row_lo, row_hi = ctx.seg
                check(lib.gsr_render_backward(P, W, H, _ptr(ranges), _ptr(point_list), _ptr(means2D),
                                              _ptr(conic_opacity), _ptr(rgb), _ptr(mask), _ptr(bg), _ptr(final_T),
                                              _ptr(n_contrib), _ptr(g_out), _ptr(record), _ptr(out_img),
                                              _ptr(seg_ws), seg_bytes, row_lo, row_hi, 1 if record_is_zero else 0,
                                              _ptr(acc64), _ptr(touched), _stream()), "gsr_render_backward")
            if _CAPTURE[0] is not None:
                _CAPTURE[0].stamp("bwd1", id(cap_stats))
            if timing != "off":
                ev1.record(current_stream(dev))
        stats = ctx.cuda_args.get("stats_collector") if isinstance(ctx.cuda_args, dict) else None
        if stats is not None and timing != "off":
            f0, f1 = ctx.fwd_events
            if timing == "sync":
                ev1.synchronize()
                _last_backward_ms = float(ev0.elapsed_time(ev1))
                stats["forward_render_time"] = float(f0.elapsed_time(f1))
                stats["backward_render_time"] = _last_backward_ms
            else:
                if timing == "deferred":
                    stats["_fwd_events"] = (f0, f1)
                    stats["_bwd_events"] = (ev0, ev1)
                if f1.query():
                    stats["forward_render_time"] = float(f0.elapsed_time(f1))
                pend = getattr(_RenderGaussians, "_pending", None)
                if pend is not None and pend[1].query():
                    _last_backward_ms = float(pend[0].elapsed_time(pend[1]))
                _RenderGaussians._pending = (ev0, ev1)
                stats["backward_render_time"] = float(_last_backward_ms)
        return d_means2D, d_conic_opacity, d_rgb, None, None, None, None, None, None


_INVDEPTH_KEY = "_gsr_invdepth"


class _RenderInvDepth(torch.autograd.Function):

    @staticmethod
    def forward(ctx, means2D, conic_opacity, depths, view):
        if _CAPTURE[0] is not None:
            raise RuntimeError("diff_gaussian_rasterization: the inverse-depth map is not available under graph capture "
                               "(it needs the view's final lists)")
        ranges, point_list, mask, band, final_T, n_contrib, W, H = view
        means2D, conic_opacity = _f32c(means2D, "means2D"), _f32c(conic_opacity, "conic_opacity")
        depths = _f32c(depths, "depths")
        P = means2D.shape[0]
        if conic_opacity.shape[0] != P or depths.numel() != P:
            raise ValueError(f"render_invdepth: means2D, conic_opacity and depths must have the {P} rows of the view")
        dev = means2D.device
        out = torch.empty((H, W), dtype=torch.float32, device=dev)
        with _on(dev), kernel_timer.range("composite_invdepth", P=P):
            check(lib.gsr_render_invdepth(P, W, H, _ptr(ranges), _ptr(point_list), _ptr(means2D), _ptr(conic_opacity),
                                          _ptr(depths), _ptr(mask), _ptr(n_contrib), band[0], band[1], _ptr(out),
                                          _stream()), "gsr_render_invdepth")
        ctx.view = view
        ctx.save_for_backward(means2D, conic_opacity, depths, out)
        return out

    @staticmethod
# ... 909 lines not shown
```

### grendel-gs_amd/diff_gaussian_rasterization/_lib.py

```python
import ctypes
import os

_HERE = os.path.dirname(os.path.abspath(__file__))
LIB_PATH = os.environ.get("GSRASTER_LIB") or os.path.join(_HERE, "libgsraster.so")

c_int, c_float, c_void_p, c_size_t, c_int64 = (ctypes.c_int, ctypes.c_float, ctypes.c_void_p, ctypes.c_size_t,
                                                ctypes.c_int64)

_K11_ADAM_PREFIX = ([c_int] * 4 + [c_void_p, c_void_p, c_float] + [c_void_p] * 5 + [c_int, c_int] + [c_void_p] * 6 +
                    [c_int] + [c_void_p] * 7 + [c_float])

SIGNATURES = {
    "gsr_error_string": (ctypes.c_char_p, [c_int]),
    "gsr_abi_version": (c_int, []),
    "gsr_get_block_xy": (c_int, [ctypes.POINTER(c_int)] * 3),
    "gsr_preprocess_forward": (c_int, [c_int, c_int, c_int, c_void_p, c_void_p, c_float, c_void_p, c_void_p, c_void_p,
                                       c_void_p, c_void_p, c_void_p, c_int, c_int, c_float, c_float, c_void_p,
                                       c_void_p, c_void_p, c_void_p, c_void_p, c_void_p, c_void_p, c_void_p]),
    "gsr_preprocess_backward": (c_int, [c_int, c_int, c_int, c_void_p, c_void_p, c_float, c_void_p, c_void_p,
                                        c_void_p, c_void_p, c_void_p, c_int, c_int, c_float, c_float] +
                                [c_void_p] * 6 + [c_int] + [c_void_p] * 6),
    "gsr_set_antialiasing": (c_int, [c_int]),
    "gsr_preprocess_backward_aa": (c_int, [c_int, c_int, c_int, c_void_p, c_void_p, c_float, c_void_p, c_void_p,
                                           c_void_p, c_void_p, c_void_p, c_void_p, c_int, c_int, c_float, c_float] +
# ... 30 lines not shown
                                              c_void_p, c_void_p, c_void_p, c_void_p, c_void_p]),
    "gsr_stamp": (c_int, [c_void_p, c_void_p, ctypes.c_uint32, ctypes.c_uint32, ctypes.c_uint32, c_void_p]),
    "gsr_band_mask": (c_int, [c_int, c_int, c_int, c_void_p, c_int, c_void_p, c_void_p]),
    "gsr_l1_ssim_finalize": (c_int, [c_int, c_void_p, c_float, c_float, c_float, c_float, c_void_p, c_void_p]),
    "gsr_image_metrics_num_partials": (c_int, [c_int, c_int, c_int]),
    "gsr_image_metrics": (c_int, [c_int, c_int, c_int, c_void_p, c_int64, c_void_p, c_int64, c_int, c_int, c_int,
                                  c_void_p, c_void_p, c_void_p]),
    "gsr_image_metrics_finalize": (c_int, [c_int, c_int, c_void_p, c_void_p, c_void_p]),
    "gsr_exchange_need": (c_int, [c_int, c_int, c_int, c_int, c_int, c_void_p, c_void_p, c_void_p, c_void_p, c_void_p,
                                  c_void_p]),
    "gsr_exchange_chunks": (c_size_t, [c_int]),
    "gsr_exchange_count": (c_int, [c_int] * 7 + [c_void_p] * 6),
    "gsr_exchange_pack": (c_int, [c_int] * 9 + [c_void_p] * 8 + [c_int64, c_void_p, c_void_p, c_void_p]),
    "gsr_exchange_pack_slab": (c_int, [c_int] * 9 + [c_void_p] * 9 + [c_int64, c_void_p, c_void_p, c_void_p]),
    "gsr_exchange_unpack": (c_int, [c_int64] + [c_void_p] * 7),
    "gsr_zero_async": (c_int, [c_void_p, c_size_t, c_void_p]),
    "gsr_scatter_add_rows": (c_int, [c_int64, c_void_p, c_void_p, c_void_p, c_void_p]),
    "gsr_knn_workspace_bytes": (c_size_t, [c_int]),
    "gsr_knn_mean_dist2": (c_int, [c_int, c_void_p, c_void_p, c_void_p, c_size_t, c_void_p]),
    "gsr_densify_stats": (c_int, [c_int64, c_void_p, c_void_p, c_int64, c_void_p, c_void_p, c_void_p, c_void_p]),
    "gsr_group_rows_bytes": (c_size_t, [c_int64]),
    "gsr_group_rows": (c_int, [c_int64, c_int, c_void_p, c_void_p, c_void_p, c_void_p, c_size_t, c_void_p]),
    "gsr_gather_rows": (c_int, [c_int64, c_void_p, c_int, c_void_p, c_void_p, c_void_p, c_void_p, c_void_p,
                                c_void_p]),
    "gsr_scatter_rows": (c_int, [c_int64, c_void_p, c_int, c_void_p, c_void_p, c_void_p, c_void_p, c_void_p,
                                 c_void_p]),
    "gsr_densify_plan_bytes": (c_size_t, [c_int64]),
    "gsr_densify_plan": (c_int, [c_int64, c_void_p, c_void_p, c_void_p, c_void_p, c_void_p, c_size_t, c_void_p]),
    "gsr_densify_move": (c_int, [c_int64, c_void_p, c_void_p, c_int64, c_int64, c_int64, c_int64, c_int, c_int] +
                         [c_void_p] * 7 + [c_int64, c_void_p, c_void_p, c_void_p]),
    "gsr_mcmc_relocate_bytes": (c_size_t, [c_int64]),
    "gsr_mcmc_relocate_plan": (c_int, [c_int64, c_int64, c_void_p, c_float, ctypes.c_uint64, ctypes.c_uint32, c_void_p,
                                       c_void_p, c_void_p, c_void_p, c_size_t, c_void_p]),
    "gsr_mcmc_relocate_apply": (c_int, [c_int64, c_int64, c_void_p, c_void_p, c_void_p, c_float, c_int, c_int] +
                                [c_void_p] * 5),
    "gsr_mcmc_noise": (c_int, [c_int64, c_void_p, c_void_p, c_void_p, c_void_p, c_float, c_void_p, ctypes.c_uint64,
                               ctypes.c_uint32, c_void_p]),
    "gsr_mcmc_normals": (c_int, [c_int64, ctypes.c_uint64, ctypes.c_uint32, c_void_p, c_void_p]),
    "gsr_mcmc_reg_grad": (c_int, [c_int64, c_void_p, c_void_p, c_float, c_float, c_void_p, c_void_p, c_void_p]),
    "gsr_adam_step": (c_int, [c_int64, c_void_p, c_void_p, c_void_p, c_void_p, ctypes.c_double, ctypes.c_double,
                              ctypes.c_double, ctypes.c_double, c_int64, c_float, c_void_p]),
    "gsr_adam_step_multi": (c_int, [c_int] + [c_void_p] * 10 + [c_float, c_void_p]),
    "gsr_preprocess_forward_raw": (c_int, [c_int, c_int, c_int, c_void_p, c_void_p, c_float] + [c_void_p] * 7 +
                                   [c_int, c_int, c_float, c_float] + [c_void_p] * 8),
    "gsr_preprocess_backward_raw": (c_int, [c_int, c_int, c_int, c_void_p, c_void_p, c_float] + [c_void_p] * 7 +
                                    [c_int, c_int, c_float, c_float] + [c_void_p] * 6 + [c_int] + [c_void_p] * 7),
    "gsr_preprocess_forward_raw_batched": (c_int, [c_int, c_int, c_int, c_int, c_void_p, c_void_p, c_float] +
                                           [c_void_p] * 5 + [c_int, c_int] + [c_void_p] * 8),
    "gsr_preprocess_backward_raw_batched": (c_int, [c_int, c_int, c_int, c_int, c_void_p, c_void_p, c_float] +
                                            [c_void_p] * 5 + [c_int, c_int] + [c_void_p] * 6 + [c_int] +
                                            [c_void_p] * 7),
    "gsr_preprocess_backward_adam_raw_batched": (c_int, _K11_ADAM_PREFIX + [c_void_p, c_void_p]),
    "gsr_preprocess_backward_adam_raw_batched_dyn": (c_int, _K11_ADAM_PREFIX + [c_void_p] * 4),
    "gsr_sparse_step_workspace_bytes": (c_size_t, [c_int]),
    "gsr_preprocess_backward_adam_raw_batched_sparse": (c_int, _K11_ADAM_PREFIX + [c_void_p, c_void_p, c_void_p,
                                                                                    c_size_t, c_void_p, c_void_p,
                                                                                    c_void_p]),
    "gsr_preprocess_backward_cams_bytes": (c_size_t, [c_int, c_int]),
    "gsr_preprocess_backward_cams": (c_int, [c_int, c_int, c_int, c_int, c_void_p, c_void_p, c_int, c_void_p, c_int,
                                             c_void_p, c_int, c_int] + [c_void_p] * 6 + [c_int, c_void_p, c_size_t,
                                                                                         c_void_p, c_void_p]),
    "gsr_bin_total_offset": (c_size_t, [c_int, c_int, c_int]),
    "gsr_bin_segments_offset": (c_size_t, [c_int, c_int, c_int]),
    "gsr_bin_speculative_async": (c_int, [c_int, c_int, c_int, c_void_p, c_void_p, c_void_p, c_void_p, c_void_p,
                                          c_void_p, c_size_t, c_int64, c_void_p, c_size_t, c_void_p, c_void_p,
                                          ctypes.POINTER(ctypes.c_uint32), ctypes.POINTER(c_int), c_void_p]),
    "gsr_set_bin_persistent": (c_int, [c_int]),
    "gsr_set_tile_cull": (c_int, [c_int]),
    "gsr_set_bin_rowmajor": (c_int, [c_int]),
    "gsr_bin_persist_status": (c_int, [ctypes.POINTER(ctypes.c_uint32)]),
    "gsr_bin_timeline": (c_int, [c_int, c_void_p, c_int, ctypes.POINTER(c_int)]),
    "gsr_flag_if_greater": (c_int, [c_void_p, ctypes.c_uint32, c_void_p, ctypes.c_uint32, c_void_p, c_void_p]),
    "gsr_render_seg_bytes": (c_size_t, [c_int, c_int]),
    "gsr_render_forward": (c_int, [c_int, c_int, c_int] + [c_void_p] * 11 + [c_size_t, c_int, c_int, c_void_p, c_size_t,
                                                                           c_void_p]),
    "gsr_render_backward": (c_int, [c_int, c_int, c_int] + [c_void_p] * 13 + [c_size_t, c_int, c_int, c_int, c_void_p,
                                                                            c_void_p, c_void_p]),
    "gsr_composite_walked": (c_int, [ctypes.POINTER(ctypes.c_ulonglong), c_int]),
    "gsr_render_contrib": (c_int, [c_int, c_int, c_int] + [c_void_p] * 6 + [c_int, c_int] + [c_void_p] * 4),
    "gsr_contrib_merge_rows": (c_int, [c_int64] + [c_void_p] * 8),
    "gsr_render_invdepth": (c_int, [c_int, c_int, c_int] + [c_void_p] * 7 + [c_int, c_int, c_void_p, c_void_p]),
    "gsr_render_invdepth_backward": (c_int, [c_int, c_int, c_int] + [c_void_p] * 10 + [c_int, c_int] + [c_void_p] * 3),
    "gsr_depth_backward_means3d": (c_int, [c_int] + [c_void_p] * 3 + [c_int, c_void_p, c_int, c_void_p]),
    "gsr_publish_flag": (c_int, [c_void_p, c_void_p, c_void_p, ctypes.c_uint32, c_void_p]),
    "gsr_exchange_check": (c_int, [c_void_p, c_void_p, c_int, c_int, c_int, ctypes.c_uint64, c_int, c_void_p,
                                   ctypes.c_uint32, ctypes.c_uint32, c_void_p, c_void_p]),
    "gsr_activate_forward": (c_int, [c_int, c_int] + [c_void_p] * 10),
    "gsr_activate_backward": (c_int, [c_int, c_int] + [c_void_p] * 13),
}

ABI_VERSION = 15


def _load():
    if not os.path.exists(LIB_PATH):
        raise ImportError(
            f"{LIB_PATH} not found: the gfx950 HIP library has not been built "
            "(run `python __graft_entry__.py build` or `python grendel-gs_amd/csrc/build.py`). "
            "There is no CPU or PyTorch fallback for this operator."
        )
    lib = ctypes.CDLL(LIB_PATH)
    for name, (res, args) in SIGNATURES.items():
        fn = getattr(lib, name)
        fn.restype = res
        fn.argtypes = args
    if lib.gsr_abi_version() != ABI_VERSION:
        raise ImportError(f"{LIB_PATH}: ABI version {lib.gsr_abi_version()} != expected {ABI_VERSION}; rebuild")
    return lib


lib = _load()


def check(code, what):
    if code != 0:
        msg = lib.gsr_error_string(code)
        raise RuntimeError(f"{what} failed: {msg.decode() if msg else code} (code {code})")
```

### grendel-gs_amd/gaussian_renderer/__init__.py

```python
import math
import os

import numpy as np
import torch
import torch.distributed as dist

import utils.general_utils as utils
from diff_gaussian_rasterization import GaussianRasterizationSettings, GaussianRasterizer

import diff_gaussian_rasterization as _dgr

import contextlib

_NULL = contextlib.nullcontext()


def _keep_grad_view(t):
    import weakref
    ref, first = weakref.ref(t), [True]

    def hook(g):
        x = ref()
        if x is not None:
            x.grad = g if first[0] else x.grad + g
            first[0] = False

    t.register_hook(hook)

N_DIFF = 9
N_AUX = 2


def get_cuda_args_final(strategy, mode="train"):
    args = utils.get_args()
    iteration = utils.get_cur_iter()
    if mode == "train":
        for x in range(args.bsz):
            if (iteration + x) % args.log_interval == 1:
                iteration += x
                break
    elif mode == "test":
        iteration = -1
    else:
        raise ValueError("mode should be train or test.")
    ca = {
        "mode": mode,
        "world_size": str(utils.WORLD_SIZE),
        "global_rank": str(utils.GLOBAL_RANK),
        "local_rank": str(utils.LOCAL_RANK),
        "mp_world_size": str(strategy.world_size),
        "mp_rank": str(strategy.rank),
        "log_folder": args.log_folder,
        "log_interval": str(args.log_interval),
        "iteration": str(iteration),
        "zhx_debug": str(args.zhx_debug),
        "zhx_time": str(args.zhx_time),
        "avoid_pixel_all2all": False,
        "stats_collector": {},
    }
    if _INVDEPTH[0]:
        ca["invdepth"] = True
    return ca


_INVDEPTH = [os.environ.get("GSR_INVDEPTH", "0") not in ("", "0")]


def set_invdepth(on):
    _INVDEPTH[0] = bool(on)


def get_invdepth():
    return _INVDEPTH[0]


class _InvDepthNoGrad(torch.autograd.Function):
# ... 580 lines not shown
            pose_grad = True
            packed.append(_dgr.pack_camera(rast.raster_settings))
            continue
        rs_k = rast.raster_settings
        key = (float(rs_k.tanfovx), float(rs_k.tanfovy)) + tuple(
            (t.data_ptr(), t._version) for t in (rs_k.viewmatrix, rs_k.projmatrix, rs_k.campos))
        cached = getattr(camera, "_gsr_packed", None)
        if cached is None or cached[0] != key or cached[1].device != raw[0].device:
            cached = (key, _dgr.pack_camera(rast.raster_settings))
            try:
                camera._gsr_packed = cached
            except AttributeError:
                pass
        packed.append(cached[1])
    rs0 = rasterizers[0].raster_settings
    if len(packed) == 1:
        cams_block = packed[0].view(1, -1)
    elif pose_grad or _dgr.capturing() is not None:
        cams_block = torch.stack(packed)
    else:
        skey = tuple(id(t) for t in packed)
        hit = _CAMERA_BLOCKS.get(skey)
        if hit is not None and all(a is b and a._version == v for a, b, v in zip(hit[1], packed, hit[2])):
            cams_block = hit[0]
        else:
            cams_block = torch.stack(packed)
            if len(_CAMERA_BLOCKS) > 1024:
                _CAMERA_BLOCKS.clear()
            _CAMERA_BLOCKS[skey] = (cams_block, tuple(packed), tuple(t._version for t in packed))
    m2_all, rgb_all, co_all, radii_all, depths_all = _dgr.preprocess_gaussians_raw_batched(
        *raw, cams_block, pc.active_sh_degree,
        scaling_modifier, rs0.image_width, rs0.image_height, tanfov0=(rs0.tanfovx, rs0.tanfovy),
        cuda_args_list=cuda_args_list)
    for k in range(len(rasterizers)):
        means2D = m2_all[k]
        if mode == "train":
            _keep_grad_view(means2D)
        params.append([means2D, rgb_all[k], co_all[k], radii_all[k], depths_all[k]])
    if timers is not None:
        timers.stop("forward_preprocess_gaussians")

    pkg = {
        "batched_locally_preprocessed_mean2D": [p[0] for p in params],
        "batched_locally_preprocessed_visibility_filter": _LazyPerCamera([p[3] for p in params], lambda r: r > 0),
        "batched_locally_preprocessed_radii": [p[3] for p in params],
        "batched_rasterizers": rasterizers,
        "batched_cuda_args": cuda_args_list,
    }
    W = utils.DEFAULT_GROUP.size()
    if W == 1 and not (_EXCHANGE_OPTIONS["forced"] and dist.is_initialized()):
        redistributed = tuple([p[c] for p in params] for c in range(5))
        sizes = [[[p[0].shape[0] for p in params]]]
        _fill(pkg, redistributed, sizes)
        if _INVDEPTH[0]:
            pkg["_invdepth_xyz"] = raw[0]
        return pkg
    if W * len(params) > 512:
        raise ValueError(f"world size x batch size = {W * len(params)} exceeds the 512 (destination, camera) segments "
                         "one exchange launch carries (include/gsraster.h: gsr_exchange_count)")
    if timers is not None:
        timers.start("forward_all_to_all_communication")
    mine = [k for k, st in enumerate(batched_strategies) if utils.GLOBAL_RANK in st.gpu_ids]

    def exchange(known=None):
        *redistributed, sizes, (events, token), pending = _batched_exchange_final(
            [p[0] for p in params], rgb_all, co_all, radii_all, depths_all, rasterizers, batched_strategies,
            speculate=False if _legacy else None, pipeline=False if _legacy else None, _known=known)
        _fill(pkg, redistributed, sizes)
        pkg["_exchange_events"] = events
        for ca in cuda_args_list:
            ca.pop("_exchange_token", None)
        if token is not None and mine:
            cuda_args_list[mine[-1]]["_exchange_token"] = token
        pkg["_exchange_token"] = token
        pkg.pop("_exchange_pending", None)
        if pending is not None:
            planner, chunkcnt, counts, lazy, staged = pending
            rendered = [(g, k) for k, st in enumerate(batched_strategies) for g in st.gpu_ids]

            def verify():
                if pkg.get("_exchange_pending") is None:
                    return True
                pkg.pop("_exchange_pending")
                m, fitted = planner.resolve(staged)
                lazy._v = m.tolist()
                recv_rows = m.sum(axis=0).tolist()
                ok = fitted and all(recv_rows[g][k] >= 10 for (g, k) in rendered)
                planner.note(redone=not ok)
                if ok:
                    return True
                exchange_stats["redone"] += 1
                exchange(known=(chunkcnt, counts, lazy._v))
                return False

            lazy._resolver = verify
            pkg["_exchange_pending"] = verify

    exchange()
    if timers is not None:
        timers.stop("forward_all_to_all_communication")
    return pkg


def _fill(pkg, redistributed, sizes):
    for name, value in zip(("means2D", "rgb", "conic_opacity", "radii", "depths"), redistributed):
        pkg[f"batched_{name}_redistributed"] = value
# ... 189 lines not shown
```

### include/gsraster.h

```cpp
#ifndef GSRASTER_H
#define GSRASTER_H

#include <stddef.h>
#include <stdint.h>

#ifdef __cplusplus
extern "C" {
#endif

#define GSR_BLOCK_X 16
#define GSR_BLOCK_Y 16
#define GSR_ONE_DIM_BLOCK 256

#define GSR_EINVAL (-1)
#define GSR_ENOSPACE (-2)
#define GSR_ERETRY (-3)
#define GSR_EFAULT (-4)

typedef void *gsr_stream_t;

const char *gsr_error_string(int code);

int gsr_abi_version(void);

// ... 29 lines not shown
size_t gsr_bin_prepare_bytes(int P, int width, int height);
int gsr_bin_prepare(int P, int width, int height, const float *means2D, const float *depths, const int32_t *radii,
                    const float *conic_opacity, const uint8_t *compute_locally, void *prep, size_t prep_bytes,
                    int64_t *num_rendered_host, gsr_stream_t stream);
size_t gsr_bin_sort_bytes(int P, int64_t num_rendered, int width, int height);
int gsr_bin_sort(int P, int width, int height, const uint8_t *compute_locally, const void *prep,
                 int64_t num_rendered, void *scratch, size_t scratch_bytes, uint32_t *point_list, int32_t *ranges,
                 gsr_stream_t stream);
int gsr_set_depth_tie_order(int mode);
int gsr_bin_prepare_async(int P, int width, int height, const float *means2D, const float *depths, const int32_t *radii,
                          const float *conic_opacity, const uint8_t *compute_locally, void *prep, size_t prep_bytes,
                          uint32_t *ticket, gsr_stream_t stream);
int gsr_bin_count_wait(uint32_t ticket, int64_t *num_rendered_host, gsr_stream_t stream);
int64_t gsr_bin_sort_capacity(int P, size_t scratch_bytes, int width, int height);
int gsr_bin_speculative_async(int P, int width, int height, const float *means2D, const float *depths,
                              const int32_t *radii, const float *conic_opacity, const uint8_t *compute_locally, void *prep,
                              size_t prep_bytes, int64_t capacity, void *scratch, size_t scratch_bytes,
                              uint32_t *point_list, int32_t *ranges, uint32_t *ticket, int *sorted, gsr_stream_t stream);
int gsr_set_bin_persistent(int mode);
int gsr_set_bin_rowmajor(int mode);
int gsr_set_tile_cull(int mode);
int gsr_bin_persist_status(uint32_t *out4);
int gsr_bin_timeline(int which, unsigned long long *out, int max_words, int *grid);
size_t gsr_bin_total_offset(int P, int width, int height);
size_t gsr_bin_segments_offset(int P, int width, int height);

int gsr_stamp(const uint32_t *seq_dev, uint64_t *host_ring_pinned, uint32_t slots, uint32_t per_slot, uint32_t index,
              gsr_stream_t stream);
int gsr_band_mask(int grid_x, int grid_y, int B, const int32_t *band_rows_dev, int stride_words, uint8_t *mask,
                  gsr_stream_t stream);
int gsr_publish_flag(const uint32_t *flag_dev, const uint32_t *seq_dev, uint32_t *host_ring_pinned, uint32_t slots,
                     gsr_stream_t stream);
int gsr_flag_if_greater(const uint32_t *value_dev, uint32_t limit, uint32_t *flag_dev, uint32_t bit,
                        uint32_t *host_copy_pinned, gsr_stream_t stream);
int gsr_exchange_check(const int32_t *all_counts_dev, const int32_t *caps_dev, int W, int B, int me,
                       uint64_t rendered_mask, int few, uint32_t *flag_dev, uint32_t bit_over, uint32_t bit_few,
                       int32_t *host_copy_pinned, gsr_stream_t stream);
int gsr_bin_sort_bounded(int P, int width, int height, const uint8_t *compute_locally, const void *prep,
                         int64_t capacity, void *scratch, size_t scratch_bytes, uint32_t *point_list, int32_t *ranges,
                         gsr_stream_t stream);

size_t gsr_render_seg_bytes(int width, int height);
int gsr_render_forward(int P, int width, int height, const int32_t *ranges, const uint32_t *point_list,
                       const float *means2D, const float *conic_opacity, const float *rgb,
                       const uint8_t *compute_locally, const float *bg, float *out_color, float *final_T,
                       int32_t *n_contrib, void *seg_ws, size_t seg_bytes, int row_lo, int row_hi, void *zero_ptr,
                       size_t zero_bytes, gsr_stream_t stream);
int gsr_render_backward(int P, int width, int height, const int32_t *ranges, const uint32_t *point_list,
                        const float *means2D, const float *conic_opacity, const float *rgb,
                        const uint8_t *compute_locally, const float *bg, const float *final_T,
                        const int32_t *n_contrib, const float *dL_dpixels, float *dL_record, const float *out_color,
                        void *seg_ws, size_t seg_bytes, int row_lo, int row_hi, int record_is_zero, double *acc64,
                        uint8_t *touched, gsr_stream_t stream);
int gsr_composite_walked(unsigned long long *out2, int reset);

int gsr_render_contrib(int P, int width, int height, const int32_t *ranges, const uint32_t *point_list,
                       const float *means2D, const float *conic_opacity, const uint8_t *compute_locally,
                       const int32_t *n_contrib, int row_lo, int row_hi, int64_t *hits, float *wmax, double *wsum,
                       gsr_stream_t stream);
int gsr_contrib_merge_rows(int64_t n, const int32_t *idx, const int64_t *src_hits, const float *src_wmax,
                           const double *src_wsum, int64_t *dst_hits, float *dst_wmax, double *dst_wsum,
                           gsr_stream_t stream);

int gsr_render_invdepth(int P, int width, int height, const int32_t *ranges, const uint32_t *point_list,
                        const float *means2D, const float *conic_opacity, const float *depths,
                        const uint8_t *compute_locally, const int32_t *n_contrib, int row_lo, int row_hi,
                        float *invdepth, gsr_stream_t stream);
int gsr_render_invdepth_backward(int P, int width, int height, const int32_t *ranges, const uint32_t *point_list,
                                 const float *means2D, const float *conic_opacity, const float *depths,
                                 const uint8_t *compute_locally, const int32_t *n_contrib, const float *final_T,
                                 const float *invdepth, const float *dL_dinvdepth, int row_lo, int row_hi,
                                 float *dL_record, double *acc64, gsr_stream_t stream);
int gsr_depth_backward_means3d(int P, const int32_t *radii, const float *viewmatrix, const float *dL_ddepth,
                               int row_stride, float *dL_dmeans3D, int overwrite, gsr_stream_t stream);

int gsr_l1_ssim_num_partials(int channels, int rows, int width);
int gsr_l1_ssim_forward(int channels, int rows, int width, const float *image, int64_t image_channel_stride,
                        const uint8_t *gt, float *partials, float *dm_dmu1, float *dm_dE11, float *dm_dE12,
                        gsr_stream_t stream);
int gsr_l1_ssim_backward(int channels, int rows, int width, const float *image, int64_t image_channel_stride,
                         const uint8_t *gt, const float *dm_dmu1, const float *dm_dE11, const float *dm_dE12,
                         const float *grad_l1_sum, const float *grad_ssim_sum, float scale_l1, float scale_ssim,
                         float *grad_image, int64_t grad_channel_stride, gsr_stream_t stream);
int gsr_l1_ssim_forward_band(int channels, int rows_capacity, int width, const float *image, int64_t image_channel_stride,
                             const uint8_t *gt, float *partials, float *dm_dmu1, float *dm_dE11, float *dm_dE12,
                             const int32_t *band_rows, gsr_stream_t stream);
int gsr_l1_ssim_backward_band(int channels, int rows_capacity, int width, const float *image,
                              int64_t image_channel_stride, const uint8_t *gt, const float *dm_dmu1, const float *dm_dE11,
                              const float *dm_dE12, const float *grad_l1_sum, const float *grad_ssim_sum, float scale_l1,
                              float scale_ssim, float *grad_image, int64_t grad_channel_stride, const int32_t *band_rows,
                              gsr_stream_t stream);
int gsr_l1_ssim_finalize(int num_partials, const float *partials, float c_l1, float c_ssim, float bias, float inv_n,
                         float *out3, gsr_stream_t stream);

int gsr_l1_ssim_forward_exposure(int channels, int rows_capacity, int width, const float *image,
                                 int64_t image_channel_stride, const uint8_t *gt, float *partials, float *dm_dmu1,
                                 float *dm_dE11, float *dm_dE12, const int32_t *band_rows, const float *exposure,
                                 gsr_stream_t stream);
int gsr_l1_ssim_exposure_num_partials(int rows, int width);
int gsr_l1_ssim_backward_exposure(int channels, int rows_capacity, int width, const float *image,
                                  int64_t image_channel_stride, const uint8_t *gt, const float *dm_dmu1,
                                  const float *dm_dE11, const float *dm_dE12, const float *grad_l1_sum,
                                  const float *grad_ssim_sum, float scale_l1, float scale_ssim, float *grad_image,
                                  int64_t grad_channel_stride, const int32_t *band_rows, const float *exposure,
                                  float *exposure_partials, float *grad_exposure, gsr_stream_t stream);

// ... 97 lines not shown
int gsr_preprocess_backward_raw(int P, int sh_degree, int sh_coeffs, const float *xyz, const float *scaling,
                                float scale_modifier, const float *rotation, const float *features_dc,
                                const float *features_rest, const float *opacity, const float *viewmatrix,
                                const float *projmatrix, const float *campos, int width, int height, float tanfovx,
                                float tanfovy, const int32_t *radii, const float *cov3D, const uint8_t *clamped,
                                const float *dL_dmeans2D, const float *dL_dconic_opacity, const float *dL_drgb,
                                int grad_row_stride, float *dL_dxyz, float *dL_dscaling, float *dL_drotation, float *dL_dfeatures_dc,
                                float *dL_dfeatures_rest, float *dL_dopacity, gsr_stream_t stream);

int gsr_preprocess_forward_raw_batched(int P, int B, int sh_degree, int sh_coeffs, const float *xyz,
                                       const float *scaling, float scale_modifier, const float *rotation,
                                       const float *features_dc, const float *features_rest, const float *opacity,
                                       const float *cams, int width, int height, float *means2D, float *depths,
                                       int32_t *radii, float *cov3D, float *conic_opacity, float *rgb,
                                       uint8_t *clamped, gsr_stream_t stream);
int gsr_preprocess_backward_raw_batched(int P, int B, int sh_degree, int sh_coeffs, const float *xyz,
                                        const float *scaling, float scale_modifier, const float *rotation,
                                        const float *features_dc, const float *features_rest, const float *opacity,
                                        const float *cams, int width, int height, const int32_t *radii,
                                        const float *cov3D, const uint8_t *clamped, const float *dL_dmeans2D,
                                        const float *dL_dconic_opacity, const float *dL_drgb, int grad_row_stride, float *dL_dxyz,
                                        float *dL_dscaling, float *dL_drotation, float *dL_dfeatures_dc,
                                        float *dL_dfeatures_rest, float *dL_dopacity, gsr_stream_t stream);

size_t gsr_preprocess_backward_cams_bytes(int P, int B);
int gsr_preprocess_backward_cams(int P, int B, int sh_degree, int sh_coeffs, const float *means3D, const float *sh_dc,
                                 int sh_dc_stride, const float *sh_rest, int sh_rest_stride, const float *cams,
                                 int width, int height, const int32_t *radii, const float *cov3D,
                                 const uint8_t *clamped, const float *dL_dmeans2D, const float *dL_dconic_opacity,
                                 const float *dL_drgb, int grad_row_stride, void *workspace, size_t workspace_bytes,
                                 float *dL_dcams, gsr_stream_t stream);

int gsr_preprocess_backward_adam_raw_batched(int P, int B, int sh_degree, int sh_coeffs, float *xyz, float *scaling,
                                             float scale_modifier, float *rotation, float *features_dc,
                                             float *features_rest, float *opacity, const float *cams, int width,
                                             int height, const int32_t *radii, const float *cov3D,
                                             const uint8_t *clamped, const float *dL_dmeans2D,
                                             const float *dL_dconic_opacity, const float *dL_drgb,
                                             int grad_row_stride, float *const *exp_avgs, float *const *exp_avg_sqs,
                                             const double *lrs, const double *beta1s, const double *beta2s,
                                             const double *epss, const int64_t *steps, float grad_scale,
                                             const float *tanfov0, gsr_stream_t stream);
int gsr_preprocess_backward_adam_raw_batched_dyn(int P, int B, int sh_degree, int sh_coeffs, float *xyz, float *scaling,
                                                 float scale_modifier, float *rotation, float *features_dc,
                                                 float *features_rest, float *opacity, const float *cams, int width,
                                                 int height, const int32_t *radii, const float *cov3D,
                                                 const uint8_t *clamped, const float *dL_dmeans2D,
                                                 const float *dL_dconic_opacity, const float *dL_drgb,
                                                 int grad_row_stride, float *const *exp_avgs,
                                                 float *const *exp_avg_sqs, const double *lrs, const double *beta1s,
                                                 const double *beta2s, const double *epss, const int64_t *steps,
                                                 float grad_scale, const float *tanfov0, const float *dyn_dev,
                                                 const uint32_t *skip_flag_dev, gsr_stream_t stream);

size_t gsr_sparse_step_workspace_bytes(int P);
int gsr_preprocess_backward_adam_raw_batched_sparse(int P, int B, int sh_degree, int sh_coeffs, float *xyz,
                                                    float *scaling, float scale_modifier, float *rotation,
                                                    float *features_dc, float *features_rest, float *opacity,
                                                    const float *cams, int width, int height, const int32_t *radii,
                                                    const float *cov3D, const uint8_t *clamped,
                                                    const float *dL_dmeans2D, const float *dL_dconic_opacity,
                                                    const float *dL_drgb, int grad_row_stride,
                                                    float *const *exp_avgs, float *const *exp_avg_sqs,
                                                    const double *lrs, const double *beta1s, const double *beta2s,
                                                    const double *epss, const int64_t *steps, float grad_scale,
                                                    const float *dyn_dev, const uint32_t *skip_flag_dev,
                                                    void *workspace, size_t workspace_bytes, uint8_t *active_out,
                                                    uint32_t *num_active_dev, gsr_stream_t stream);

int gsr_activate_forward(int N, int sh_rest, const float *scaling, const float *rotation, const float *opacity,
                         const float *features_dc, const float *features_rest, float *scales, float *rotations,
                         float *opacities, float *shs, gsr_stream_t stream);
int gsr_activate_backward(int N, int sh_rest, const float *rotation, const float *scales, const float *opacities,
                          const float *g_scales, const float *g_rotations, const float *g_opacities,
                          const float *g_shs, float *d_scaling, float *d_rotation, float *d_opacity,
                          float *d_features_dc, float *d_features_rest, gsr_stream_t stream);

#ifdef __cplusplus
}
#endif
#endif
```

Measured before the change: 833.8.

## Defer float rounding of render-backward gradients into fused preprocess-backward Adam kernel

Render backward can now leave per-Gaussian gradients in the f64 accumulator plus a touched mask, with no float record. The fused preprocess-backward+Adam kernel reads the f64 sums directly for up to 8 cameras, and a lazy materialize path runs only when something else needs the float record. This removes the record_from_f64 conversion kernel and one write plus read of the float gradient buffer per view. In exchange it adds deferred-state bookkeeping in Python and a more complex contract about record lifetime.

```diff
diff --git a/grendel-gs_amd/csrc/api.hip b/grendel-gs_amd/csrc/api.hip
--- a/grendel-gs_amd/csrc/api.hip
+++ b/grendel-gs_amd/csrc/api.hip
@@ -174,7 +174,33 @@
         return GSR_EINVAL;
     return gsr_launch_composite_backward(P, width, height, ranges, point_list, means2D, conic_opacity, rgb,
                                          compute_locally, bg, final_T, n_contrib, dL_dpixels, dL_record, out_color,
-                                         seg_ws, seg_bytes, row_lo, row_hi, record_is_zero ? 1 : 0, acc64, touched,
+                                         seg_ws, seg_bytes, row_lo, row_hi, record_is_zero ? 1 : 0, acc64, touched, 1,
+                                         reinterpret_cast<hipStream_t>(stream));
+}
+
+int gsr_render_backward_sums(int P, int width, int height, const int32_t *ranges, const uint32_t *point_list,
+                             const float *means2D, const float *conic_opacity, const float *rgb,
+                             const uint8_t *compute_locally, const float *bg, const float *final_T,
+                             const int32_t *n_contrib, const float *dL_dpixels, const float *out_color, void *seg_ws,
+                             size_t seg_bytes, int row_lo, int row_hi, double *acc64, uint8_t *touched,
+                             gsr_stream_t stream) {
+    if (P < 0 || width <= 0 || height <= 0) return GSR_EINVAL;
+    if (P == 0) return 0;
+    if (!ranges || !compute_locally || !bg || !final_T || !n_contrib || !dL_dpixels || !means2D || !conic_opacity ||
+        !rgb || !acc64 || !touched)
+        return GSR_EINVAL;
+    return gsr_launch_composite_backward(P, width, height, ranges, point_list, means2D, conic_opacity, rgb,
+                                         compute_locally, bg, final_T, n_contrib, dL_dpixels, nullptr, out_color,
+                                         seg_ws, seg_bytes, row_lo, row_hi, 1, acc64, touched, 0,
+                                         reinterpret_cast<hipStream_t>(stream));
+}
+
+int gsr_render_record_materialize(int P, const double *acc64, const uint8_t *touched, float *dL_record,
+                                  int record_is_zero, gsr_stream_t stream) {
+    if (P < 0) return GSR_EINVAL;
+    if (P == 0) return 0;
+    if (!acc64 || !touched || !dL_record) return GSR_EINVAL;
+    return gsr_launch_record_materialize(P, acc64, touched, dL_record, record_is_zero ? 1 : 0,
                                          reinterpret_cast<hipStream_t>(stream));
 }
 
diff --git a/grendel-gs_amd/csrc/common.h b/grendel-gs_amd/csrc/common.h
--- a/grendel-gs_amd/csrc/common.h
+++ b/grendel-gs_amd/csrc/common.h
@@ -135,7 +135,10 @@
                                   const uint8_t *compute_locally, const float *bg, const float *final_T,
                                   const int32_t *n_contrib, const float *dL_dpixels, float *dL_record,
                                   const float *out_color, void *seg_ws, size_t seg_bytes, int row_lo, int row_hi,
-                                  int record_is_zero, double *acc64, uint8_t *touched, hipStream_t stream);
+                                  int record_is_zero, double *acc64, uint8_t *touched, int round_record,
+                                  hipStream_t stream);
+int gsr_launch_record_materialize(int P, const double *acc64, const uint8_t *touched, float *dL_record,
+                                  int record_is_zero, hipStream_t stream);
 int gsr_launch_composite_contrib(int P, int W, int H, const int32_t *ranges, const uint32_t *point_list,
                                  const float *means2D, const float *conic_opacity, const uint8_t *compute_locally,
                                  const int32_t *n_contrib, int row_lo, int row_hi, int64_t *hits, float *wmax,
diff --git a/grendel-gs_amd/csrc/composite.hip b/grendel-gs_amd/csrc/composite.hip
--- a/grendel-gs_amd/csrc/composite.hip
+++ b/grendel-gs_amd/csrc/composite.hip
@@ -1,3 +1,6 @@
+#include <atomic>
+#include <cstdlib>
+
 #include "common.h"
 #include "composite_math.h"
 
@@ -831,7 +834,9 @@
                                   const uint8_t *compute_locally, const float *bg, const float *final_T,
                                   const int32_t *n_contrib, const float *dL_dpixels, float *dL_record,
                                   const float *out_color, void *seg_ws, size_t seg_bytes, int row_lo, int row_hi,
-                                  int record_is_zero, double *acc64, uint8_t *touched, hipStream_t stream) {
+                                  int record_is_zero, double *acc64, uint8_t *touched, int round_record,
+                                  hipStream_t stream) {
+    if (!round_record && (!record_is_zero || !touched)) return GSR_EINVAL;
     if (!record_is_zero) {
         touched = nullptr;
         GSR_HIP(hipMemsetAsync(acc64, 0, sizeof(double) * 9 * (size_t)P, stream));
@@ -848,6 +853,7 @@
                        reinterpret_cast<const float4 *>(conic_opacity), rgb, compute_locally, bg, final_T, n_contrib,
                        dL_dpixels, acc64, seg, b.band_first, b.band_tiles, touched);
     GSR_LAUNCH_CHECK();
+    if (!round_record) return 0;
     if (touched)
         hipLaunchKernelGGL(record_from_f64_touched_kernel, dim3((unsigned)((P + 255) / 256)), dim3(256), 0, stream,
                            acc64, dL_record, touched, P);
@@ -857,3 +863,29 @@
     GSR_LAUNCH_CHECK();
     return 0;
 }
+
+int gsr_launch_record_materialize(int P, const double *acc64, const uint8_t *touched, float *dL_record,
+                                  int record_is_zero, hipStream_t stream) {
+    if (P == 0) return 0;
+    if (!record_is_zero) GSR_HIP(hipMemsetAsync(dL_record, 0, sizeof(float) * 9 * (size_t)P, stream));
+    hipLaunchKernelGGL(record_from_f64_touched_kernel, dim3((unsigned)((P + 255) / 256)), dim3(256), 0, stream, acc64,
+                       dL_record, touched, P);
+    GSR_LAUNCH_CHECK();
+    return 0;
+}
+
+static std::atomic<int> g_deferred_rounding{-1};
+extern "C" int gsr_set_deferred_rounding(int mode) {
+    if (mode < -1 || mode > 1) return GSR_EINVAL;
+    g_deferred_rounding.store(mode, std::memory_order_relaxed);
+    return 0;
+}
+extern "C" int gsr_deferred_rounding(void) {
+    const int mode = g_deferred_rounding.load(std::memory_order_relaxed);
+    if (mode >= 0) return mode;
+    static const int env_mode = [] {
+        const char *e = getenv("GSR_DEFER_ROUNDING");
+        return (e && *e == '0') ? 0 : 1;
+    }();
+    return env_mode;
+}
diff --git a/grendel-gs_amd/csrc/preprocess.hip b/grendel-gs_amd/csrc/preprocess.hip
--- a/grendel-gs_amd/csrc/preprocess.hip
+++ b/grendel-gs_amd/csrc/preprocess.hip
@@ -758,6 +758,61 @@
     return in;
 }
 
+struct GradRecord {
+    const float *means2D, *conic_opacity, *rgb;
+    int gstride;
+};
+constexpr int K11_SUMS_CAMS = 8;
+struct GradSums {
+    const double *acc[K11_SUMS_CAMS];
+    const uint8_t *flags[K11_SUMS_CAMS];
+};
+#ifndef GSR_K11_SUMS_COV_ALWAYS
+#define GSR_K11_SUMS_COV_ALWAYS 0
+#endif
+
+__device__ __forceinline__ K11In k11_load_sums(size_t i, int32_t rad, uint8_t flag, const float *__restrict__ xyz,
+                                               const float *__restrict__ scaling, const float *__restrict__ rotation,
+                                               const float *__restrict__ f_dc, const float *__restrict__ opacity,
+                                               const float *__restrict__ cov3D, const uint8_t *__restrict__ clamped,
+                                               const double *__restrict__ acc) {
+    K11In in;
+#pragma unroll
+    for (int e = 0; e < 3; e++) {
+        in.p[e] = xyz[3 * i + e];
+        in.sc[e] = scaling[3 * i + e];
+        in.dc[e] = f_dc[3 * i + e];
+        in.cl[e] = GSR_K11_SUMS_COV_ALWAYS ? clamped[3 * i + e] : (uint8_t)0;
+        in.grgb[e] = 0.f;
+    }
+    in.op = opacity[i];
+    in.q = *reinterpret_cast<const float4 *>(rotation + 4 * i);
+#pragma unroll
+    for (int e = 0; e < 6; e++) in.cv[e] = GSR_K11_SUMS_COV_ALWAYS ? cov3D[6 * i + e] : 0.f;
+    in.gco = make_float4(0.f, 0.f, 0.f, 0.f);
+    in.g2 = make_float2(0.f, 0.f);
+    __builtin_amdgcn_sched_barrier(0);
+    const bool live = flag && rad > 0;
+    in.rad = live ? rad : 0;
+    if (live) {
+        const double *a = acc + 9 * i;
+        double v[9];
+#pragma unroll
+        for (int k = 0; k < 9; k++) v[k] = a[k];
+        if (!GSR_K11_SUMS_COV_ALWAYS) {
+#pragma unroll
+            for (int e = 0; e < 6; e++) in.cv[e] = cov3D[6 * i + e];
+#pragma unroll
+            for (int e = 0; e < 3; e++) in.cl[e] = clamped[3 * i + e];
+        }
+        in.g2 = make_float2((float)v[0], (float)v[1]);
+#pragma unroll
+        for (int e = 0; e < 3; e++) in.grgb[e] = (float)v[2 + e];
+        in.gco = make_float4((float)v[5], (float)v[6], (float)v[7], (float)v[8]);
+    }
+    return in;
+}
+
 template <bool RAW, bool ADAM>
 __device__ __forceinline__ void k11_opacity_out(float op, float g, const int i, float (&sp)[14], float (&sg)[14],
                                                 float *__restrict__ dL_dopacities) {
@@ -963,24 +1018,35 @@
                                                   dL_dmeans3D, dL_dscales, dL_drotations, dL_dshs, dL_dopacities);
 }
 
-template <int DEG, bool AA>
-__global__ void __launch_bounds__(K11_BLOCK, K11_WAVES_PER_EU)
-preprocess_backward_adam_kernel(int P, float *__restrict__ xyz, float *__restrict__ scaling, float scale_modifier,
-                                float *__restrict__ rotation, float *__restrict__ f_dc, float *__restrict__ f_rest,
-                                float *__restrict__ opacity, const float *__restrict__ view,
-                                const float *__restrict__ proj, const float *__restrict__ campos, int W, int H,
-                                float tanfovx, float tanfovy, const int32_t *__restrict__ radii,
-                                const float *__restrict__ cov3D, const uint8_t *__restrict__ clamped,
-                                const float *__restrict__ dL_dmeans2D, const float *__restrict__ dL_dconic_opacity,
-                                const float *__restrict__ dL_drgb, int gstride, const K11Adam ad_in) {
+struct GradNone {};
+template <int DEG, bool AA, typename GRAD>
+__device__ __forceinline__ void
+preprocess_backward_adam_body(int P, float *__restrict__ xyz, float *__restrict__ scaling, float scale_modifier,
+                              float *__restrict__ rotation, float *__restrict__ f_dc, float *__restrict__ f_rest,
+                              float *__restrict__ opacity, const float *__restrict__ view,
+                              const float *__restrict__ proj, const float *__restrict__ campos, int W, int H,
+                              float tanfovx, float tanfovy, const int32_t *__restrict__ radii,
+                              const float *__restrict__ cov3D, const uint8_t *__restrict__ clamped,
+                              const float *__restrict__ dL_dmeans2D, const float *__restrict__ dL_dconic_opacity,
+                              const float *__restrict__ dL_drgb, int gstride, const GRAD &sums, const K11Adam &ad_in) {
     if (ad_in.skip && *ad_in.skip) return;
     const K11Adam ad = k11_adam_resolve(ad_in);
     const int i = blockIdx.x * blockDim.x + threadIdx.x;
     __shared__ float s_rest[K11_BLOCK * REST_W];
     const size_t ic = (size_t)min(i, P - 1);
+    int32_t rad = 0;
+    uint8_t flag = 0;
+    if constexpr (std::is_same<GRAD, GradSums>::value) {
+        rad = radii[ic];
+        flag = sums.flags[0][ic];
+    }
     RestStage st = rest_stage_issue(f_rest, P);
-    const K11In in = k11_load<true>(ic, xyz, scaling, rotation, f_dc, opacity, radii, cov3D, clamped, dL_dmeans2D,
-                                    dL_dconic_opacity, dL_drgb, gstride);
+    K11In in;
+    if constexpr (std::is_same<GRAD, GradSums>::value)
+        in = k11_load_sums(ic, rad, flag, xyz, scaling, rotation, f_dc, opacity, cov3D, clamped, sums.acc[0]);
+    else
+        in = k11_load<true>(ic, xyz, scaling, rotation, f_dc, opacity, radii, cov3D, clamped, dL_dmeans2D,
+                            dL_dconic_opacity, dL_drgb, gstride);
     __builtin_amdgcn_sched_barrier(0);
     rest_stage_commit(s_rest, st, f_rest, P);
     __syncthreads();
@@ -994,6 +1060,33 @@
     rest_adam_out(s_rest, f_rest, ad, P);
     __syncthreads();
     k11_adam_small_lds(s_rest, ad, P, i, xyz, scaling, rotation, f_dc, opacity, sp, sg);
+}
+template <int DEG, bool AA>
+__global__ void __launch_bounds__(K11_BLOCK, K11_WAVES_PER_EU)
+preprocess_backward_adam_kernel(int P, float *__restrict__ xyz, float *__restrict__ scaling, float scale_modifier,
+                                float *__restrict__ rotation, float *__restrict__ f_dc, float *__restrict__ f_rest,
+                                float *__restrict__ opacity, const float *__restrict__ view,
+                                const float *__restrict__ proj, const float *__restrict__ campos, int W, int H,
+                                float tanfovx, float tanfovy, const int32_t *__restrict__ radii,
+                                const float *__restrict__ cov3D, const uint8_t *__restrict__ clamped,
+                                const float *__restrict__ dL_dmeans2D, const float *__restrict__ dL_dconic_opacity,
+                                const float *__restrict__ dL_drgb, int gstride, const K11Adam ad_in) {
+    preprocess_backward_adam_body<DEG, AA>(P, xyz, scaling, scale_modifier, rotation, f_dc, f_rest, opacity, view, proj,
+                                           campos, W, H, tanfovx, tanfovy, radii, cov3D, clamped, dL_dmeans2D,
+                                           dL_dconic_opacity, dL_drgb, gstride, GradNone{}, ad_in);
+}
+template <int DEG, bool AA>
+__global__ void __launch_bounds__(K11_BLOCK, K11_WAVES_PER_EU)
+preprocess_backward_adam_sums_kernel(int P, float *__restrict__ xyz, float *__restrict__ scaling, float scale_modifier,
+                                     float *__restrict__ rotation, float *__restrict__ f_dc,
+                                     float *__restrict__ f_rest, float *__restrict__ opacity,
+                                     const float *__restrict__ view, const float *__restrict__ proj,
+                                     const float *__restrict__ campos, int W, int H, float tanfovx, float tanfovy,
+                                     const int32_t *__restrict__ radii, const float *__restrict__ cov3D,
+                                     const uint8_t *__restrict__ clamped, const GradSums sums, const K11Adam ad_in) {
+    preprocess_backward_adam_body<DEG, AA>(P, xyz, scaling, scale_modifier, rotation, f_dc, f_rest, opacity, view, proj,
+                                           campos, W, H, tanfovx, tanfovy, radii, cov3D, clamped, nullptr, nullptr,
+                                           nullptr, 0, sums, ad_in);
 }
 
 constexpr int CAM_STRIDE = 40;
@@ -1119,6 +1212,35 @@
     c.g2 = grad_ld2(dL_dmeans2D, o, gstride);
     return c;
 }
+__device__ __forceinline__ K11CamSH k11_cam_load_sh_sums(size_t o, bool live, const uint8_t *__restrict__ clamped,
+                                                         const double *__restrict__ a) {
+    K11CamSH c;
+    c.rad = live ? 1 : 0;
+#pragma unroll
+    for (int e = 0; e < 3; e++) {
+        c.grgb[e] = 0.f;
+        c.cl[e] = 0;
+    }
+    if (live) {
+#pragma unroll
+        for (int e = 0; e < 3; e++) {
+            c.grgb[e] = (float)a[2 + e];
+            c.cl[e] = clamped[3 * o + e];
+        }
+    }
+    return c;
+}
+__device__ __forceinline__ K11CamGeo k11_cam_load_geo_sums(bool live, const double *__restrict__ a) {
+    K11CamGeo c;
+    c.rad = live ? 1 : 0;
+    c.gco = make_float4(0.f, 0.f, 0.f, 0.f);
+    c.g2 = make_float2(0.f, 0.f);
+    if (live) {
+        c.g2 = make_float2((float)a[0], (float)a[1]);
+        c.gco = make_float4((float)a[5], (float)a[6], (float)a[7], (float)a[8]);
+    }
+    return c;
+}
 
 struct DenseRows {};
 struct ListRows {
@@ -1200,7 +1322,7 @@
     }
 }
 
-template <int DEG, bool ADAM, bool AA, typename ROWS = DenseRows>
+template <int DEG, bool ADAM, bool AA, typename ROWS = DenseRows, bool SUMS = false>
 __device__ __forceinline__ void
 preprocess_backward_batched_body(int P, int B, int M, const float *__restrict__ xyz,
                                    const float *__restrict__ scaling, float scale_modifier,
@@ -1214,9 +1336,10 @@
                                    float *__restrict__ dL_dxyz, float *__restrict__ dL_dscaling,
                                    float4 *__restrict__ dL_drotation, float *__restrict__ dL_ddc,
                                    float *__restrict__ dL_drest, float *__restrict__ dL_dopacity, const K11Adam &ad,
-                                   const ROWS rows = ROWS{}) {
+                                   const ROWS rows = ROWS{}, const GradSums *sums = nullptr) {
     constexpr bool LIST = std::is_same<ROWS, ListRows>::value;
     static_assert(!LIST || ADAM, "ListRows is the sparse K11 + Adam update (and takes M == 16)");
+    static_assert(!SUMS || (ADAM && !LIST), "GradSums (B <= K11_SUMS_CAMS) feeds the fused dense kernel only");
     __shared__ float s_rest[K11_BLOCK * REST_W];
     __shared__ uint32_t s_rows[LIST ? K11_BLOCK : 1];
     const bool staged = M == 16;
@@ -1224,6 +1347,7 @@
     int i, nrows = 0;
     size_t ic;
     RestStage st;
+    uint32_t live = 0;
     if constexpr (LIST) {
         const size_t first = (size_t)blockIdx.x * K11_BLOCK;
         nrows = (int)min((size_t)K11_BLOCK, (size_t)rows.count - first);
@@ -1234,12 +1358,29 @@
     } else {
         i = blockIdx.x * blockDim.x + threadIdx.x;
         ic = (size_t)min(i, P - 1);
-        if (staged) st = rest_stage_issue(f_rest, P);
+        if constexpr (SUMS) {
+            int32_t rd[K11_SUMS_CAMS];
+            uint8_t fl[K11_SUMS_CAMS];
+#pragma unroll
+            for (int u = 0; u < K11_SUMS_CAMS; u++) {
+                const int c = min(u, B - 1);
+                rd[u] = radii[(size_t)c * P + ic];
+                fl[u] = sums->flags[c][ic];
+            }
+            if (staged) st = rest_stage_issue(f_rest, P);
+            __builtin_amdgcn_sched_barrier(0);
+#pragma unroll
+            for (int u = 0; u < K11_SUMS_CAMS; u++) live |= (u < B && fl[u] && rd[u] > 0) ? 1u << u : 0u;
+        } else if (staged) st = rest_stage_issue(f_rest, P);
     }
     const float p[3] = {xyz[3 * ic], xyz[3 * ic + 1], xyz[3 * ic + 2]};
     float cvr[6];
 #pragma unroll
-    for (int e = 0; e < 6; e++) cvr[e] = cov3D[6 * ic + e];
+    for (int e = 0; e < 6; e++) cvr[e] = SUMS ? 0.f : cov3D[6 * ic + e];
+    if (SUMS && live) {
+#pragma unroll
+        for (int e = 0; e < 6; e++) cvr[e] = cov3D[6 * ic + e];
+    }
     const float dc[3] = {f_dc[3 * ic], f_dc[3 * ic + 1], f_dc[3 * ic + 2]};
     const float oraw = opacity[ic];
     const float4 qraw = *reinterpret_cast<const float4 *>(rotation + 4 * ic);
@@ -1250,8 +1391,15 @@
 #pragma unroll
         for (int u = 0; u < K11_CAMQ; u++) {
             const size_t o = (size_t)min(u, B - 1) * P + ic;
-            shq[u] = k11_cam_load_sh(o, radii, clamped, dL_drgb, gstride);
-            geoq[u] = k11_cam_load_geo(o, radii, dL_dmeans2D, dL_dconic_opacity, gstride);
+            if constexpr (SUMS) {
+                const int c = min(u, B - 1);
+                const double *a = sums->acc[c] + 9 * ic;
+                shq[u] = k11_cam_load_sh_sums(o, (live >> c) & 1u, clamped, a);
+                geoq[u] = k11_cam_load_geo_sums((live >> c) & 1u, a);
+            } else {
+                shq[u] = k11_cam_load_sh(o, radii, clamped, dL_drgb, gstride);
+                geoq[u] = k11_cam_load_geo(o, radii, dL_dmeans2D, dL_dconic_opacity, gstride);
+            }
         }
     }
     __builtin_amdgcn_sched_barrier(0);
@@ -1290,8 +1438,15 @@
         if constexpr (!LIST) {
 #pragma unroll
             for (int u = 0; u + 1 < K11_CAMQ; u++) shq[u] = shq[u + 1];
-            if (bc + K11_CAMQ < B)
-                shq[K11_CAMQ - 1] = k11_cam_load_sh((size_t)(bc + K11_CAMQ) * P + i, radii, clamped, dL_drgb, gstride);
+            if (bc + K11_CAMQ < B) {
+                if constexpr (SUMS)
+                    shq[K11_CAMQ - 1] =
+                        k11_cam_load_sh_sums((size_t)(bc + K11_CAMQ) * P + i, (live >> (bc + K11_CAMQ)) & 1u, clamped,
+                                             sums->acc[bc + K11_CAMQ] + 9 * (size_t)i);
+                else
+                    shq[K11_CAMQ - 1] =
+                        k11_cam_load_sh((size_t)(bc + K11_CAMQ) * P + i, radii, clamped, dL_drgb, gstride);
+            }
         }
         if (cin.rad <= 0) continue;
         if (staged) asm volatile("" ::: "memory");
@@ -1328,9 +1483,14 @@
         if constexpr (!LIST) {
 #pragma unroll
             for (int u = 0; u + 1 < K11_CAMQ; u++) geoq[u] = geoq[u + 1];
-            if (bc + K11_CAMQ < B)
-                geoq[K11_CAMQ - 1] = k11_cam_load_geo((size_t)(bc + K11_CAMQ) * P + i, radii, dL_dmeans2D,
-                                                      dL_dconic_opacity, gstride);
+            if (bc + K11_CAMQ < B) {
+                if constexpr (SUMS)
+                    geoq[K11_CAMQ - 1] = k11_cam_load_geo_sums((live >> (bc + K11_CAMQ)) & 1u,
+                                                               sums->acc[bc + K11_CAMQ] + 9 * (size_t)i);
+                else
+                    geoq[K11_CAMQ - 1] = k11_cam_load_geo((size_t)(bc + K11_CAMQ) * P + i, radii, dL_dmeans2D,
+                                                          dL_dconic_opacity, gstride);
+            }
         }
         if (cin.rad <= 0) continue;
         const float *cp = cams + (size_t)bc * CAM_STRIDE;
@@ -1448,6 +1608,21 @@
                                                     opacity, cams, W, H, radii, cov3D, clamped, dL_dmeans2D,
                                                     dL_dconic_opacity, dL_drgb, gstride, nullptr, nullptr, nullptr,
                                                     nullptr, nullptr, nullptr, ad);
+}
+template <int DEG, bool AA>
+__global__ void __launch_bounds__(K11_BLOCK, K11B_WAVES_PER_EU)
+preprocess_backward_adam_batched_sums_kernel(int P, int B, float *__restrict__ xyz, float *__restrict__ scaling,
+                                             float scale_modifier, float *__restrict__ rotation,
+                                             float *__restrict__ f_dc, float *__restrict__ f_rest,
+                                             float *__restrict__ opacity, const float *__restrict__ cams, int W, int H,
+                                             const int32_t *__restrict__ radii, const float *__restrict__ cov3D,
+                                             const uint8_t *__restrict__ clamped, const GradSums sums,
+                                             const K11Adam ad_in) {
+    if (ad_in.skip && *ad_in.skip) return;
+    const K11Adam ad = k11_adam_resolve(ad_in);
+    preprocess_backward_batched_body<DEG, true, AA, DenseRows, true>(
+        P, B, 16, xyz, scaling, scale_modifier, rotation, f_dc, f_rest, opacity, cams, W, H, radii, cov3D, clamped,
+        nullptr, nullptr, nullptr, 0, nullptr, nullptr, nullptr, nullptr, nullptr, nullptr, ad, DenseRows{}, &sums);
 }
 
 constexpr int SA_CBLOCK = 256;
@@ -1870,6 +2045,52 @@
     return false;
 }
 
+template <typename SRC>
+static int k11_adam_launch(int P, int B, int sh_degree, float *xyz, float *scaling, float scale_modifier, float *rotation,
+                           float *features_dc, float *features_rest, float *opacity, const float *cams, int width,
+                           int height, const int32_t *radii, const float *cov3D, const uint8_t *clamped, const SRC &src,
+                           const K11Adam &ad, const float *tanfov0, gsr_stream_t stream) {
+    uintptr_t al = (uintptr_t)features_rest | (uintptr_t)rotation;
+    for (int t = 0; t < 6; t++) al |= (uintptr_t)ad.m[t] | (uintptr_t)ad.v[t];
+    if (al & 15) return GSR_EINVAL;
+    const dim3 grid(gsr_div_up(P, K11_BLOCK)), block(K11_BLOCK);
+    const int aa = gsr_antialiasing_mode();
+    if (B == 1 && tanfov0) {
+        if constexpr (std::is_same<SRC, GradSums>::value) {
+            GSR_DISPATCH_DEG_AA(sh_degree, aa,
+                             hipLaunchKernelGGL((preprocess_backward_adam_sums_kernel<DEG, AA>), grid, block, 0,
+                                                reinterpret_cast<hipStream_t>(stream), P, xyz, scaling, scale_modifier,
+                                                rotation, features_dc, features_rest, opacity, cams, cams + 16,
+                                                cams + 32, width, height, tanfov0[0], tanfov0[1], radii, cov3D, clamped,
+                                                src, ad));
+        } else {
+            GSR_DISPATCH_DEG_AA(sh_degree, aa,
+                             hipLaunchKernelGGL((preprocess_backward_adam_kernel<DEG, AA>), grid, block, 0,
+                                                reinterpret_cast<hipStream_t>(stream), P, xyz, scaling, scale_modifier,
+                                                rotation, features_dc, features_rest, opacity, cams, cams + 16,
+                                                cams + 32, width, height, tanfov0[0], tanfov0[1], radii, cov3D, clamped,
+                                                src.means2D, src.conic_opacity, src.rgb, src.gstride, ad));
+        }
+        GSR_LAUNCH_CHECK();
+        return 0;
+    }
+    if constexpr (std::is_same<SRC, GradSums>::value) {
+        GSR_DISPATCH_DEG_AA(sh_degree, aa,
+                         hipLaunchKernelGGL((preprocess_backward_adam_batched_sums_kernel<DEG, AA>), grid, block, 0,
+                                            reinterpret_cast<hipStream_t>(stream), P, B, xyz, scaling, scale_modifier,
+                                            rotation, features_dc, features_rest, opacity, cams, width, height, radii,
+                                            cov3D, clamped, src, ad));
+    } else {
+        GSR_DISPATCH_DEG_AA(sh_degree, aa,
+                         hipLaunchKernelGGL((preprocess_backward_adam_batched_kernel<DEG, AA>), grid, block, 0,
+                                            reinterpret_cast<hipStream_t>(stream), P, B, xyz, scaling, scale_modifier,
+                                            rotation, features_dc, features_rest, opacity, cams, width, height, radii,
+                                            cov3D, clamped, src.means2D, src.conic_opacity, src.rgb, src.gstride, ad));
+    }
+    GSR_LAUNCH_CHECK();
+    return 0;
+}
+
 extern "C" int gsr_preprocess_backward_adam_raw_batched(
     int P, int B, int sh_degree, int sh_coeffs, float *xyz, float *scaling, float scale_modifier, float *rotation,
     float *features_dc, float *features_rest, float *opacity, const float *cams, int width, int height,
@@ -1899,28 +2120,35 @@
                            dL_dmeans2D, dL_dconic_opacity, dL_drgb},
                       exp_avgs, exp_avg_sqs, lrs, beta1s, beta2s, epss, steps, grad_scale, dyn_dev, skip_flag_dev))
         return GSR_EINVAL;
-    uintptr_t al = (uintptr_t)features_rest | (uintptr_t)rotation;
-    for (int t = 0; t < 6; t++) al |= (uintptr_t)ad.m[t] | (uintptr_t)ad.v[t];
-    if (al & 15) return GSR_EINVAL;
-    const dim3 grid(gsr_div_up(P, K11_BLOCK)), block(K11_BLOCK);
-    const int aa = gsr_antialiasing_mode();
-    if (B == 1 && tanfov0) {
-        GSR_DISPATCH_DEG_AA(sh_degree, aa,
-                         hipLaunchKernelGGL((preprocess_backward_adam_kernel<DEG, AA>), grid, block, 0,
-                                            reinterpret_cast<hipStream_t>(stream), P, xyz, scaling, scale_modifier,
-                                            rotation, features_dc, features_rest, opacity, cams, cams + 16, cams + 32,
-                                            width, height, tanfov0[0], tanfov0[1], radii, cov3D, clamped, dL_dmeans2D,
-                                            dL_dconic_opacity, dL_drgb, grad_row_stride, ad));
-        GSR_LAUNCH_CHECK();
-        return 0;
-    }
-    GSR_DISPATCH_DEG_AA(sh_degree, aa,
-                     hipLaunchKernelGGL((preprocess_backward_adam_batched_kernel<DEG, AA>), grid, block, 0,
-                                        reinterpret_cast<hipStream_t>(stream), P, B, xyz, scaling, scale_modifier,
-                                        rotation, features_dc, features_rest, opacity, cams, width, height, radii,
-                                        cov3D, clamped, dL_dmeans2D, dL_dconic_opacity, dL_drgb, grad_row_stride, ad));
-    GSR_LAUNCH_CHECK();
-    return 0;
+    return k11_adam_launch(P, B, sh_degree, xyz, scaling, scale_modifier, rotation, features_dc, features_rest, opacity,
+                           cams, width, height, radii, cov3D, clamped,
+                           GradRecord{dL_dmeans2D, dL_dconic_opacity, dL_drgb, grad_row_stride}, ad, tanfov0, stream);
+}
+
+extern "C" int gsr_preprocess_backward_adam_raw_batched_sums(
+    int P, int B, int sh_degree, int sh_coeffs, float *xyz, float *scaling, float scale_modifier, float *rotation,
+    float *features_dc, float *features_rest, float *opacity, const float *cams, int width, int height,
+    const int32_t *radii, const float *cov3D, const uint8_t *clamped, const double *const *acc64,
+    const uint8_t *const *touched, float *const *exp_avgs, float *const *exp_avg_sqs, const double *lrs,
+    const double *beta1s, const double *beta2s, const double *epss, const int64_t *steps, float grad_scale,
+    const float *tanfov0, const float *dyn_dev, const uint32_t *skip_flag_dev, gsr_stream_t stream) {
+    if (P < 0 || B < 1 || B > K11_SUMS_CAMS || sh_degree < 0 || sh_degree > 3 || sh_coeffs != 16 || width <= 0 ||
+        height <= 0)
+        return GSR_EINVAL;
+    if (P == 0) return 0;
+    if (!acc64 || !touched) return GSR_EINVAL;
+    GradSums src{};
+    for (int c = 0; c < K11_SUMS_CAMS; c++) {
+        src.acc[c] = acc64[c < B ? c : B - 1];
+        src.flags[c] = touched[c < B ? c : B - 1];
+        if (!src.acc[c] || !src.flags[c] || ((uintptr_t)src.acc[c] & 7)) return GSR_EINVAL;
+    }
+    K11Adam ad{};
+    if (k11_adam_fill(ad, {xyz, scaling, rotation, features_dc, features_rest, opacity, cams, radii, cov3D, clamped},
+                      exp_avgs, exp_avg_sqs, lrs, beta1s, beta2s, epss, steps, grad_scale, dyn_dev, skip_flag_dev))
+        return GSR_EINVAL;
+    return k11_adam_launch(P, B, sh_degree, xyz, scaling, scale_modifier, rotation, features_dc, features_rest, opacity,
+                           cams, width, height, radii, cov3D, clamped, src, ad, tanfov0, stream);
 }
 
 extern "C" size_t gsr_sparse_step_workspace_bytes(int P) {
diff --git a/grendel-gs_amd/diff_gaussian_rasterization/__init__.py b/grendel-gs_amd/diff_gaussian_rasterization/__init__.py
--- a/grendel-gs_amd/diff_gaussian_rasterization/__init__.py
+++ b/grendel-gs_amd/diff_gaussian_rasterization/__init__.py
@@ -5,6 +5,7 @@
 
 import torch
 import torch.nn as nn
+import torch.utils._pytree
 
 from . import _lib
 from ._lib import check, lib
@@ -511,6 +512,112 @@
     return base.view(B * P, 9)
 
 
+DEFER_MAX_CAMERAS = 8
+_DEFERRED = {}
+deferred_rounding_stats = {"deferred": 0, "materialized": 0, "fused_from_sums": 0}
+
+
+def set_deferred_rounding(mode):
+    code = {"env": -1, True: 1, "on": 1, False: 0, "off": 0}.get(mode)
+    if code is None:
+        raise ValueError('set_deferred_rounding: mode must be "env", True / "on" or False / "off"')
+    check(lib.gsr_set_deferred_rounding(code), "gsr_set_deferred_rounding")
+
+
+def deferred_rounding():
+    return bool(lib.gsr_deferred_rounding())
+
+
+def _defer_armed(cuda_args, P, have_flags):
+    if not (isinstance(cuda_args, dict) and cuda_args.get("_gsr_defer_record")) or not have_flags or P < 2:
+        return False
+    if _CAPTURE[0] is not None or not deferred_rounding():
+        return False
+    sink = deferred_backward_sink()
+    return sink is not None and bool(getattr(sink, "fuse_backward", False)) and not getattr(sink, "sparse", False)
+
+
+class _DeferredRecord:
+
+    def __init__(self, record, acc64, touched, stream):
+        self.record, self.acc64, self.touched, self.stream = record, acc64, touched, stream
+        self.materialized = False
+        deferred_rounding_stats["deferred"] += 1
+
+    def is_view(self, g, off, cols):
+        r = self.record
+        return g is not None and g.dtype == torch.float32 and tuple(g.shape) == (r.shape[0], cols) and \
+            g.stride() == (9, 1) and g.data_ptr() == r.data_ptr() + 4 * off
+
+    def materialize(self):
+        if self.materialized:
+            return
+        self.materialized = True
+        deferred_rounding_stats["materialized"] += 1
+        r = self.record
+        with _on(r.device):
+            if self.stream is not None:
+                cur = current_stream(r.device)
+                if cur != self.stream:
+                    cur.wait_stream(self.stream)
+            check(lib.gsr_render_record_materialize(r.shape[0], _ptr(self.acc64), _ptr(self.touched), _ptr(r), 1,
+                                                    _stream()), "gsr_render_record_materialize")
+
+
+_DEFERRED_MAX = 16
+
+
+def _register_deferred(key, entry):
+    while len(_DEFERRED) >= _DEFERRED_MAX:
+        _DEFERRED.pop(next(iter(_DEFERRED))).materialize()
+    _DEFERRED[key] = entry
+
+
+def _deferred_of(g):
+    if g is None or not _DEFERRED:
+        return None
+    p = g.data_ptr()
+    for e in _DEFERRED.values():
+        lo = e.record.data_ptr()
+        if lo <= p < lo + 36 * e.record.shape[0] and not e.materialized:
+            return e
+    return None
+
+
+def _take_deferred(key, g):
+    e = _DEFERRED.pop(key, None)
+    if e is None:
+        e = _deferred_of(g)
+        if e is not None:
+            for k in [k for k, v in _DEFERRED.items() if v is e]:
+                del _DEFERRED[k]
+    return e
+
+
+class _LazyRecordView(torch.Tensor):
+
+    @classmethod
+    def __torch_function__(cls, func, types, args=(), kwargs=None):
+        for t in torch.utils._pytree.tree_leaves((args, kwargs)):
+            e = getattr(t, "_gsr_deferred", None) if isinstance(t, _LazyRecordView) else None
+            if e is not None:
+                e.materialize()
+        with torch._C.DisableTorchFunctionSubclass():
+            out = func(*args, **(kwargs or {}))
+        return out.as_subclass(torch.Tensor) if isinstance(out, _LazyRecordView) else out
+
+
+def lazy_record_view(g):
+    e = _deferred_of(g)
+    return g if e is None else _lazy_view(g, e)
+
+
+def _lazy_view(g, entry):
+    v = torch.Tensor._make_subclass(_LazyRecordView, g)
+    v._gsr_deferred = entry
+    return v
+
+
 _DEFERRED_SINK = [None]
 
 
@@ -527,7 +634,9 @@
 
 class PendingProjectionBackward:
 
-    def __init__(self, params, cams, radii, cov3D, clamped, g_means2D, g_conic_opacity, g_rgb, gstride, meta, tanfov0):
+    def __init__(self, params, cams, radii, cov3D, clamped, g_means2D, g_conic_opacity, g_rgb, gstride, meta, tanfov0,
+                 deferred=None):
+        self.deferred = deferred
         self.params = params
         self.versions = tuple(t._version for t in params)
         self.cams, self.radii, self.cov3D, self.clamped = cams, radii, cov3D, clamped
@@ -541,14 +650,32 @@
             if cur != self.stream:
                 cur.wait_stream(self.stream)
 
+    def round_records(self):
+        entries, self.deferred = self.deferred, None
+        if entries is None:
+            return
+        self.join_stream()
+        for e in entries:
+            e.materialize()
+        if len(entries) > 1:
+            recs = [e.record for e in entries]
+            self.g_means2D = torch.stack([r[:, 0:2] for r in recs])
+            self.g_rgb = torch.stack([r[:, 2:5] for r in recs])
+            self.g_conic_opacity = torch.stack([r[:, 5:9] for r in recs])
+            self.gstride = 0
+
     def materialize(self):
         self.join_stream()
+        self.round_records()
         return _launch_k11(self.params, self.cams, self.radii, self.cov3D, self.clamped, self.g_means2D,
                            self.g_conic_opacity, self.g_rgb, self.gstride, self.meta, self.tanfov0, None)
 
     def fused_step(self, exp_avgs, exp_avg_sqs, lrs, beta1s, beta2s, epss, steps, grad_scale, cache=None,
                    sparse=False):
         self.join_stream()
+        if self.deferred is not None and (sparse or not deferred_rounding()):
+            self.round_records()
+        sums = self.deferred
         xyz, scaling, rotation, f_dc, f_rest, opacity = self.params
         deg, smod, W, H, M = self.meta[:5]
         P, B = xyz.shape[0], self.cams.shape[0]
@@ -564,12 +691,20 @@
             if (B == 1 and self.tanfov0 is not None) else None
         cap_ctx = _CAPTURE[0]
         dyn, flag = (_ptr(cap_ctx.dyn), _ptr(cap_ctx.flag)) if cap_ctx is not None else (None, None)
+        if sums is not None:
+            PB = ctypes.c_void_p * B
+            grad_args = [PB(*[e.acc64.data_ptr() for e in sums]), PB(*[e.touched.data_ptr() for e in sums])]
+        else:
+            grad_args = [_ptr(self.g_means2D), _ptr(self.g_conic_opacity), _ptr(self.g_rgb), self.gstride]
         args = [P, B, deg, M, _ptr(xyz), _ptr(scaling), smod, _ptr(rotation), _ptr(f_dc), _ptr(f_rest), _ptr(opacity),
-                _ptr(self.cams), W, H, _ptr(self.radii), _ptr(self.cov3D), _ptr(self.clamped), _ptr(self.g_means2D),
-                _ptr(self.g_conic_opacity), _ptr(self.g_rgb), self.gstride, tabs[1], tabs[2],
-                None if cap_ctx is not None else D(*lrs), tabs[3], tabs[4], tabs[5],
+                _ptr(self.cams), W, H, _ptr(self.radii), _ptr(self.cov3D), _ptr(self.clamped)] + grad_args + \
+               [tabs[1], tabs[2], None if cap_ctx is not None else D(*lrs), tabs[3], tabs[4], tabs[5],
                 None if cap_ctx is not None else I64(*steps), float(grad_scale)]
-        if sparse:
+        if sums is not None:
+            name, timed = "gsr_preprocess_backward_adam_raw_batched_sums", "preprocess_backward_adam"
+            args += [tf, dyn, flag]
+            deferred_rounding_stats["fused_from_sums"] += B
+        elif sparse:
             if cache is None:
                 cache = {}
             need = int(lib.gsr_sparse_step_workspace_bytes(P))
@@ -659,6 +794,7 @@
                 _ptr(means2D), _ptr(depths), _ptr(radii), _ptr(cov3D), _ptr(conic_opacity), _ptr(rgb), _ptr(clamped),
                 _stream()), "gsr_preprocess_forward_raw_batched")
         ctx.meta = (int(sh_degree), float(scale_modifier), int(width), int(height), M, aa)
+        ctx.m2_ptr = means2D.data_ptr()
         ctx.save_for_backward(xyz, scaling, rotation, features_dc, features_rest, opacity, cams, radii, cov3D, clamped)
         outs = []
         for k in range(B):
@@ -689,23 +825,50 @@
                     out[k].copy_(g)
             return out
 
-        if B == 1:
+        params = (xyz, scaling, rotation, f_dc, f_rest, opacity)
+        entries = [_take_deferred(ctx.m2_ptr + 8 * k * P, grads[5 * k]) if _DEFERRED else None for k in range(B)]
+        deferred = None
+        if any(e is not None for e in entries):
+            for k, e in enumerate(entries):
+                for col, (off, cols) in enumerate(((0, 2), (2, 3), (5, 4))):
+                    g = grads[5 * k + col]
+                    if e is not None and g is not None and not e.is_view(g, off, cols):
+                        raise RuntimeError(
+                            "diff_gaussian_rasterization: the rounding of a view's gradient record was deferred, but "
+                            "another gradient reached means2D / rgb / conic_opacity of that view and autograd has added "
+                            "it to the unrounded record; call set_deferred_rounding(False) for such a graph")
+            whole = all(e is not None and all(grads[5 * k + c] is not None for c in range(3))
+                        for k, e in enumerate(entries))
+            sink = deferred_backward_sink()
+            if whole and not ctx.needs_input_grad[6] and B <= DEFER_MAX_CAMERAS and M == 16 and sink is not None and \
+                    not getattr(sink, "sparse", False) and deferred_rounding() and sink.accepts(params):
+                deferred = entries
+            else:
+                for e in entries:
+                    if e is not None:
+                        e.materialize()
+        if deferred is not None and B > 1:
+            g_means2D = g_rgb = g_conic_opacity = None
+            gstride = 0
+        elif B == 1:
             g_means2D, g_rgb, g_conic_opacity, gstride = _grad_triple(grads[0], grads[1], grads[2], P, dev)
+            if deferred is not None:
+                g_means2D, g_rgb, g_conic_opacity = (_lazy_view(g, deferred[0])
+                                                     for g in (g_means2D, g_rgb, g_conic_opacity))
         else:
             rec = _batched_record(grads, B, P)
             if rec is not None:
                 g_means2D, g_rgb, g_conic_opacity, gstride = rec[:, 0:2], rec[:, 2:5], rec[:, 5:9], 9
             else:
                 g_means2D, g_rgb, g_conic_opacity, gstride = assemble(0, 2), assemble(1, 3), assemble(2, 4), 0
-        params = (xyz, scaling, rotation, f_dc, f_rest, opacity)
         d_cams = None
         if ctx.needs_input_grad[6]:
             d_cams = preprocess_backward_cameras(xyz, (f_dc, f_rest), cams, W, H, deg, radii, cov3D, clamped,
                                                  g_means2D, g_conic_opacity, g_rgb, gstride)
         sink = deferred_backward_sink()
-        if sink is not None and M == 16 and sink.accepts(params):
+        if deferred is not None or (sink is not None and M == 16 and sink.accepts(params)):
             sink.offer(PendingProjectionBackward(params, cams, radii, cov3D, clamped, g_means2D, g_conic_opacity,
-                                                 g_rgb, gstride, ctx.meta, ctx.tanfov0))
+                                                 g_rgb, gstride, ctx.meta, ctx.tanfov0, deferred))
             return (None,) * 6 + (d_cams,) + (None,) * 6
         return _launch_k11(params, cams, radii, cov3D, clamped, g_means2D, g_conic_opacity, g_rgb, gstride, ctx.meta,
                            ctx.tanfov0, ctx.cuda_args_list) + (d_cams,) + (None,) * 6
@@ -1039,6 +1202,8 @@
             lists = [point_list]
             record = acc64 = touched = None
             zero_buf, zero_bytes = None, 0
+            ctx.defer = all(ctx.needs_input_grad[:3]) and _ZERO_IN_FORWARD[0] and \
+                _defer_armed(cuda_args, P, _TOUCHED_ROWS[0])
             if any(ctx.needs_input_grad[:3]) and P > 0 and _ZERO_IN_FORWARD[0]:
                 if _TOUCHED_ROWS[0]:
                     zero_bytes = 108 * P + ((P + 15) & ~15)
@@ -1134,14 +1299,28 @@
             cap_stats = ctx.cuda_args.get("stats_collector") if isinstance(ctx.cuda_args, dict) else None
             if _CAPTURE[0] is not None:
                 _CAPTURE[0].stamp("bwd0", id(cap_stats))
+            defer = record_is_zero and getattr(ctx, "defer", False)
             with kernel_timer.range("composite_backward", P=P, D=ctx.num_rendered, **ctx.px_meta), \
                     zhx_range(ctx.cuda_args, "b10 render time"):
                 seg_ws, seg_bytes, row_lo, row_hi = ctx.seg
-                check(lib.gsr_render_backward(P, W, H, _ptr(ranges), _ptr(point_list), _ptr(means2D),
-                                              _ptr(conic_opacity), _ptr(rgb), _ptr(mask), _ptr(bg), _ptr(final_T),
-                                              _ptr(n_contrib), _ptr(g_out), _ptr(record), _ptr(out_img),
-                                              _ptr(seg_ws), seg_bytes, row_lo, row_hi, 1 if record_is_zero else 0,
-                                              _ptr(acc64), _ptr(touched), _stream()), "gsr_render_backward")
+                if defer:
+                    check(lib.gsr_render_backward_sums(P, W, H, _ptr(ranges), _ptr(point_list), _ptr(means2D),
+                                                       _ptr(conic_opacity), _ptr(rgb), _ptr(mask), _ptr(bg),
+                                                       _ptr(final_T), _ptr(n_contrib), _ptr(g_out), _ptr(out_img),
+                                                       _ptr(seg_ws), seg_bytes, row_lo, row_hi, _ptr(acc64),
+                                                       _ptr(touched), _stream()), "gsr_render_backward_sums")
+                    entry = _DeferredRecord(record, acc64, touched, current_stream(dev))
+                    if _defer_armed(ctx.cuda_args, P, True):
+                        _register_deferred(means2D.data_ptr(), entry)
+                    else:
+                        entry.materialize()
+                else:
+                    check(lib.gsr_render_backward(P, W, H, _ptr(ranges), _ptr(point_list), _ptr(means2D),
+                                                  _ptr(conic_opacity), _ptr(rgb), _ptr(mask), _ptr(bg), _ptr(final_T),
+                                                  _ptr(n_contrib), _ptr(g_out), _ptr(record), _ptr(out_img),
+                                                  _ptr(seg_ws), seg_bytes, row_lo, row_hi,
+                                                  1 if record_is_zero else 0, _ptr(acc64), _ptr(touched), _stream()),
+                          "gsr_render_backward")
             if _CAPTURE[0] is not None:
                 _CAPTURE[0].stamp("bwd1", id(cap_stats))
             if timing != "off":
diff --git a/grendel-gs_amd/diff_gaussian_rasterization/_lib.py b/grendel-gs_amd/diff_gaussian_rasterization/_lib.py
--- a/grendel-gs_amd/diff_gaussian_rasterization/_lib.py
+++ b/grendel-gs_amd/diff_gaussian_rasterization/_lib.py
@@ -106,6 +106,9 @@
                                             [c_void_p] * 7),
     "gsr_preprocess_backward_adam_raw_batched": (c_int, _K11_ADAM_PREFIX + [c_void_p, c_void_p]),
     "gsr_preprocess_backward_adam_raw_batched_dyn": (c_int, _K11_ADAM_PREFIX + [c_void_p] * 4),
+    "gsr_preprocess_backward_adam_raw_batched_sums": (c_int, [c_int] * 4 + [c_void_p, c_void_p, c_float] +
+                                                      [c_void_p] * 5 + [c_int, c_int] + [c_void_p] * 12 + [c_float] +
+                                                      [c_void_p] * 4),
     "gsr_sparse_step_workspace_bytes": (c_size_t, [c_int]),
     "gsr_preprocess_backward_adam_raw_batched_sparse": (c_int, _K11_ADAM_PREFIX + [c_void_p, c_void_p, c_void_p,
                                                                                     c_size_t, c_void_p, c_void_p,
@@ -130,6 +133,11 @@
                                                                            c_void_p]),
     "gsr_render_backward": (c_int, [c_int, c_int, c_int] + [c_void_p] * 13 + [c_size_t, c_int, c_int, c_int, c_void_p,
                                                                             c_void_p, c_void_p]),
+    "gsr_render_backward_sums": (c_int, [c_int, c_int, c_int] + [c_void_p] * 12 + [c_size_t, c_int, c_int, c_void_p,
+                                                                                 c_void_p, c_void_p]),
+    "gsr_render_record_materialize": (c_int, [c_int, c_void_p, c_void_p, c_void_p, c_int, c_void_p]),
+    "gsr_set_deferred_rounding": (c_int, [c_int]),
+    "gsr_deferred_rounding": (c_int, []),
     "gsr_composite_walked": (c_int, [ctypes.POINTER(ctypes.c_ulonglong), c_int]),
     "gsr_render_contrib": (c_int, [c_int, c_int, c_int] + [c_void_p] * 6 + [c_int, c_int] + [c_void_p] * 4),
     "gsr_contrib_merge_rows": (c_int, [c_int64] + [c_void_p] * 8),
diff --git a/grendel-gs_amd/gaussian_renderer/__init__.py b/grendel-gs_amd/gaussian_renderer/__init__.py
--- a/grendel-gs_amd/gaussian_renderer/__init__.py
+++ b/grendel-gs_amd/gaussian_renderer/__init__.py
@@ -22,6 +22,7 @@
     def hook(g):
         x = ref()
         if x is not None:
+            g = _dgr.lazy_record_view(g)
             x.grad = g if first[0] else x.grad + g
             first[0] = False
 
@@ -708,6 +709,9 @@
         redistributed = tuple([p[c] for p in params] for c in range(5))
         sizes = [[[p[0].shape[0] for p in params]]]
         _fill(pkg, redistributed, sizes)
+        if mode == "train" and not pose_grad and not _INVDEPTH[0] and len(cuda_args_list) <= _dgr.DEFER_MAX_CAMERAS:
+            for ca in cuda_args_list:
+                ca["_gsr_defer_record"] = True
         if _INVDEPTH[0]:
             pkg["_invdepth_xyz"] = raw[0]
         return pkg
diff --git a/include/gsraster.h b/include/gsraster.h
--- a/include/gsraster.h
+++ b/include/gsraster.h
@@ -105,6 +105,16 @@
                         const int32_t *n_contrib, const float *dL_dpixels, float *dL_record, const float *out_color,
                         void *seg_ws, size_t seg_bytes, int row_lo, int row_hi, int record_is_zero, double *acc64,
                         uint8_t *touched, gsr_stream_t stream);
+int gsr_render_backward_sums(int P, int width, int height, const int32_t *ranges, const uint32_t *point_list,
+                             const float *means2D, const float *conic_opacity, const float *rgb,
+                             const uint8_t *compute_locally, const float *bg, const float *final_T,
+                             const int32_t *n_contrib, const float *dL_dpixels, const float *out_color, void *seg_ws,
+                             size_t seg_bytes, int row_lo, int row_hi, double *acc64, uint8_t *touched,
+                             gsr_stream_t stream);
+int gsr_render_record_materialize(int P, const double *acc64, const uint8_t *touched, float *dL_record,
+                                  int record_is_zero, gsr_stream_t stream);
+int gsr_set_deferred_rounding(int mode);
+int gsr_deferred_rounding(void);
 int gsr_composite_walked(unsigned long long *out2, int reset);
 
 int gsr_render_contrib(int P, int width, int height, const int32_t *ranges, const uint32_t *point_list,
@@ -308,6 +318,16 @@
                                                  const double *beta2s, const double *epss, const int64_t *steps,
                                                  float grad_scale, const float *tanfov0, const float *dyn_dev,
                                                  const uint32_t *skip_flag_dev, gsr_stream_t stream);
+int gsr_preprocess_backward_adam_raw_batched_sums(int P, int B, int sh_degree, int sh_coeffs, float *xyz, float *scaling,
+                                                  float scale_modifier, float *rotation, float *features_dc,
+                                                  float *features_rest, float *opacity, const float *cams, int width,
+                                                  int height, const int32_t *radii, const float *cov3D,
+                                                  const uint8_t *clamped, const double *const *acc64,
+                                                  const uint8_t *const *touched, float *const *exp_avgs,
+                                                  float *const *exp_avg_sqs, const double *lrs, const double *beta1s,
+                                                  const double *beta2s, const double *epss, const int64_t *steps,
+                                                  float grad_scale, const float *tanfov0, const float *dyn_dev,
+                                                  const uint32_t *skip_flag_dev, gsr_stream_t stream);
 
 size_t gsr_sparse_step_workspace_bytes(int P);
 int gsr_preprocess_backward_adam_raw_batched_sparse(int P, int B, int sh_degree, int sh_coeffs, float *xyz,
```

New measurement: 842.8 (median of 6 runs). 1.1% higher.
